# jolibrain/jolineedle

Hardware: AMD Instinct MI355X
Metric: glimpse-patches/sec (448px, seq-len 20) REINFORCE step (higher is better)
Workload: dtype f32; 1 GPU; configs[2]/[3]: REINFORCE rollout, gpt-nano + yolox-nano encoder, 448px, seq-len 20, --enable-stop, 64 agents/GPU x 1 GPU, 4480x4480 synthetic images, forced non-STOP actions (S=T); global_batch=64, seq_len=20

## Files before the change

include/jnroll.h:

```cpp
#ifndef JNROLL_H
#define JNROLL_H

#include <stddef.h>
#include <stdint.h>

#ifdef __cplusplus
extern "C" {
#endif

#define JN_ABI_VERSION 2

enum {
  JN_OK = 0,
  JN_EINVAL = -1,
  JN_ENOMEM = -2,
  JN_EHIP = -3,
  JN_ENOTFOUND = -4,
  JN_ESTATE = -5
};

enum { JN_MODE_GREEDY = 0, JN_MODE_SAMPLE = 1, JN_MODE_FORCED = 2 };

enum { JN_NET_GPT_BACKBONE = 0, JN_NET_DETECTOR = 1 };

typedef struct jn_ctx jn_ctx;

typedef struct jn_config {
  int32_t struct_size;
  int32_t device;
  int32_t n_layer, n_head, n_embd;
  int32_t block_size;
  int32_t n_actions;
  int32_t patch_size;
  int32_t use_pos_emb;
  int32_t no_patch_emb;
  int32_t concat_emb;
  int32_t decoder_pos_encoding;
  int32_t pos_emb_size;
  float gpt_bb_depth, gpt_bb_width;
  int32_t gpt_bb_depthwise;
  int32_t with_detector;
  float det_depth, det_width;
  int32_t det_depthwise;
  float det_conf_threshold;
  float det_nms_threshold;
  int32_t max_batch;
  int32_t max_det_per_patch;
  int32_t act_dtype;
  int32_t gpt_wide;
} jn_config;

typedef struct jn_tensor {
  const char* name;
  const void* data;
  int32_t dtype;
  int32_t ndim;
  int64_t shape[4];
} jn_tensor;

typedef struct jn_param_info {
  char name[160];
  int32_t dtype;
  int32_t ndim;
  int64_t shape[4];
  int32_t is_buffer;
  int32_t used;
} jn_param_info;

typedef struct jn_rollout_out {
  float* rewards_dev;
  float* returns_dev;
  float* logprobs_dev;
  float* entropies_dev;
  uint8_t* masks_dev;
  uint8_t* logit_masks_dev;
  int64_t* positions_dev;
  int64_t* actions_dev;
  float* logits_dev;
  float* final_emb_dev;
  float* patches_dev;
  float* det_boxes_dev;
  int32_t* det_counts_dev;
} jn_rollout_out;

int jn_abi_version(void);
const char* jn_last_error(void);
int jn_create(const jn_config* cfg, jn_ctx** out);
int jn_destroy(jn_ctx* ctx);

int jn_param_count(const jn_ctx* ctx);
int jn_param_info_at(const jn_ctx* ctx, int index, jn_param_info* out);
int jn_debug_forward_plan(const jn_ctx* ctx, int net, int N, int train, int with_head, int first_op, int32_t* out,
                          int cap);
int jn_debug_decision_route(const jn_ctx* ctx);
int jn_load_weights(jn_ctx* ctx, const jn_tensor* tensors, size_t n);

int jn_env_init(jn_ctx* ctx, const float* images_dev, const int64_t* bboxes_dev,
                int B, int H, int W, int nb, int max_ep_len, int stop_enabled, void* stream);
int jn_env_init_u8(jn_ctx* ctx, const uint8_t* images_dev, const int64_t* bboxes_dev,
                   int B, int H, int W, int nb, int max_ep_len, int stop_enabled, void* stream);
int jn_env_reset(jn_ctx* ctx, const int64_t* positions_dev, uint64_t seed, void* stream);
int jn_env_step(jn_ctx* ctx, const int64_t* actions_dev, float* rewards_dev,
                uint8_t* terminated_dev, uint8_t* truncated_dev, void* stream);
int jn_env_state(jn_ctx* ctx, int what, void** ptr_dev);
int jn_env_patches(jn_ctx* ctx, float* out_dev, void* stream);
int jn_gather_patches(const float* images_dev, const int64_t* positions_dev, float* out_dev,
                      int B, int C, int H, int W, int P, void* stream);
int jn_gather_patches_u8(const uint8_t* images_dev, const int64_t* positions_dev, float* out_dev,
                         int B, int C, int H, int W, int P, void* stream);
int jn_gather_patches_indexed(const float* images_dev, const int64_t* image_index_dev,
                              const int64_t* positions_dev, float* out_dev, int N, int n_images,
                              int C, int H, int W, int P, void* stream);
int jn_gather_patches_indexed_u8(const uint8_t* images_dev, const int64_t* image_index_dev,
                                 const int64_t* positions_dev, float* out_dev, int N, int n_images,
                                 int C, int H, int W, int P, void* stream);

typedef struct jn_image_view {
  const void* src;
  int32_t src_u8;
  int32_t Hs, Ws;
  int32_t rot;
  int32_t ty, tx;
} jn_image_view;
int jn_env_init_views(jn_ctx* ctx, const jn_image_view* views_host, const int64_t* bboxes_dev, int B, int Hc, int Wc,
                      int nb, int max_ep_len, int stop_enabled, void* stream);
int jn_env_init_ragged(jn_ctx* ctx, const jn_image_view* views_host, const int32_t* extents_host,
                       const int64_t* bboxes_dev, int B, int Hc, int Wc, int nb, int max_ep_len, int stop_enabled,
                       void* stream);
int jn_detection_cells(const int64_t* bboxes_dev, const int32_t* extents_dev, int B, int nb, int Gh, int Gw, int P,
                       int sample_neg, uint64_t seed, int capacity, int64_t* cells_dev, int64_t* targets_dev,
                       int32_t* offsets_dev, int32_t* n_pos_dev, void* stream);
int jn_rollout_boxes_to_image(const float* det_boxes_dev, const int32_t* det_counts_dev, const int64_t* positions_dev,
                              const uint8_t* masks_dev, int B, int T, int S, int K, int P, float* out_boxes_dev,
                              int32_t* out_totals_dev, void* stream);
int jn_merge_boxes(const float* boxes_dev, const int32_t* counts_dev, int B, int Nmax, int W, int target, float threshold,
                   float* out_boxes_dev, int32_t* out_counts_dev, int32_t* rounds_dev, void* stream);
int jn_yolox_loss(const float* raw_dev, const float* targets_dev, int N, int nb, int P, int stride0, int stride1,
                  int stride2, int use_l1, float loss_scale, float* d_raw_dev, float* metrics_dev, float* scale_dev,
                  void* stream);
int jn_yolox_loss_wide(const float* raw_dev, const float* targets_dev, int N, int nb, int P, int stride0, int stride1,
                       int stride2, int use_l1, float loss_scale, float* d_raw_dev, float* metrics_dev, float* scale_dev,
                       void* stream);
int jn_postprocess(const float* raw_dev, int N, int A, float conf_threshold, float nms_threshold, float clamp_max,
                   int max_out, float* boxes_dev, int32_t* counts_dev, int32_t* stats_dev, void* stream);
int jn_postprocess_all(const float* raw_dev, int N, int A, float conf_threshold, float nms_threshold, float clamp_max,
                       int max_out, float* boxes_dev, int32_t* counts_dev, int32_t* stats_dev, void* stream);
int jn_supervised_metrics(const float* logits_dev, const int64_t* current_actions_dev, const int64_t* next_actions_dev,
                          const uint8_t* masks_dev, int B, int T, int nA, float stop_weight, int on_self_trajectory,
                          float* token_loss_out_dev, uint8_t* predicted_out_dev, float* metrics_dev, void* stream);
int jn_match_detections(const float* preds_dev, const int32_t* pred_counts_dev, int B, int Nmax, int W,
                        const float* targets_dev, const int32_t* target_counts_dev, int Mmax, int max_det,
                        double* scores_dev, int32_t* hits_dev, int32_t* sel_dev, int32_t* n_pred_dev, int32_t* n_gt_dev,
                        void* stream);
int jn_average_precision(const double* scores_dev, const int32_t* hits_dev, const int32_t* n_pred_dev,
                         const int32_t* n_gt_dev, int B, int max_det, int pooled, const double* thresholds_dev,
                         int n_thresholds, double* out_dev, void* stream);
int jn_average_precision_segments(const double* scores_dev, const int32_t* hits_dev, const int32_t* n_pred_dev,
                                  const int32_t* n_gt_dev, int U, int max_det, const int32_t* seg_offsets_dev, int NS,
                                  int max_units, const double* thresholds_dev, int n_thresholds, double* out_dev, void* stream);
int jn_pool_walk_detections(const float* det_boxes_dev, const int32_t* det_counts_dev, const int64_t* positions_dev,
                            const int32_t* walk_tokens_dev, const int32_t* walk_first_dev, const int32_t* walk_count_dev, int A,
                            int T, int S, int K_det, int NI, int max_walks, int Gh, int Gw, int max_per_cell,
                            float* cell_boxes_dev, int32_t* cell_counts_dev, int32_t* cell_stats_dev, uint8_t* visited_dev,
                            void* stream);
int jn_gather_patches_views(const jn_image_view* views_dev, int n_views, const int64_t* image_index_dev,
                            const int64_t* positions_dev, void* out_dev, int out_u8, int N, int Hc, int Wc, int P,
                            void* stream);

#define JN_AUG_NPARAM 20
int jn_augment_patches(const float* in_dev, float* out_dev, const float* params_dev, const float* noise_dev,
                       uint64_t seed, int N, int P, void* stream);

int jn_backbone_forward(jn_ctx* ctx, int net, const float* patches_dev, int N, int train,
                        float* fpn0_dev, float* fpn1_dev, float* fpn2_dev, void* stream);
int jn_read_tensor(jn_ctx* ctx, const char* name, float* host_out, size_t numel);
int jn_embed_patches(jn_ctx* ctx, const float* patches_dev, int N, float* out_dev, void* stream);
int jn_zero_grad(jn_ctx* ctx, void* stream);
int jn_backbone_backward(jn_ctx* ctx, int net, const float* patches_dev, int N, const float* g0_dev,
                         const float* g1_dev, const float* g2_dev, void* stream);
typedef struct jn_train_opts {
  int32_t struct_size;
  int32_t reward_norm;
  float ret_mean, ret_std;
  float entropy_weight;
  float loss_scale;
} jn_train_opts;

int jn_reinforce_step(jn_ctx* ctx, int mode, const int64_t* forced_actions_dev,
                      const int64_t* start_positions_dev, uint64_t seed, int stop_early,
                      const jn_train_opts* opts, const jn_rollout_out* out, float* metrics_dev, void* stream);
int jn_reinforce_forward(jn_ctx* ctx, int mode, const int64_t* forced_actions_dev, const int64_t* start_positions_dev,
                         uint64_t seed, int stop_early, const jn_rollout_out* out, void* stream);
int jn_reinforce_backward(jn_ctx* ctx, const float* dlogprobs_dev, const float* dentropies_dev, void* stream);
int jn_set_activation_slots(jn_ctx* ctx, int n);
int jn_activation_slots_info(const jn_ctx* ctx, int net, int* act_slots, int* table_slots, size_t* slot_bytes, int* replayed_steps);
int jn_replay_chunks(int S, int act_slots, int g_slots, int* t0, int* n, int cap);
int jn_debug_replay_diff(jn_ctx* ctx, int step, long long* n_diff, void* stream);
int jn_arena_segment(jn_ctx* ctx, const char* name, size_t* off, size_t* numel);
int jn_export_arena(jn_ctx* ctx, int what, float* dst_dev, size_t numel, int accumulate, void* stream);
int jn_import_arena(jn_ctx* ctx, int what, const float* src_dev, size_t numel, void* stream);

int jn_set_dropout(jn_ctx* ctx, float p, uint64_t seed);
int jn_set_freeze(jn_ctx* ctx, int freeze_detector_backbone);
int jn_optimizer_steps(jn_ctx* ctx, int group, int* steps, int set);

int jn_supervised_step(jn_ctx* ctx, const float* patches_dev, const int64_t* current_actions_dev,
                       const int64_t* next_actions_dev, const int64_t* classes_dev, const int64_t* positions_dev,
                       const uint8_t* masks_dev, int B, int T, float stop_weight, float* logits_out_dev,
                       float* metrics_dev, void* stream);
int jn_supervised_forward(jn_ctx* ctx, const float* patches_dev, const int64_t* current_actions_dev,
                          const int64_t* classes_dev, const int64_t* positions_dev, int B, int T, float* logits_out_dev,
                          float* final_emb_out_dev, void* stream);
int jn_supervised_backward(jn_ctx* ctx, const float* dlogits_dev, void* stream);
int jn_gpt_backward_route(int C, int n_head, int T, int decision_route);
int jn_gpt_attention_backward(int form, const float* QKV_dev, const float* dY_dev, int B, int n_head, int C, int Lm, int L,
                              float pdrop, uint64_t seed, int layer, int Tmax, float* ATT_dev, float* Y_dev, float* dQKV_dev,
                              void* stream);
int jn_supervised_eval(jn_ctx* ctx, const float* patches_dev, const int64_t* current_actions_dev,
                       const int64_t* next_actions_dev, const int64_t* classes_dev, const int64_t* positions_dev,
                       const uint8_t* masks_dev, int B, int T, float stop_weight, int on_self_trajectory,
                       float* logits_out_dev, float* token_loss_out_dev, uint8_t* predicted_out_dev, float* metrics_dev,
                       void* stream);
int jn_optimizer_step(jn_ctx* ctx, float lr, float weight_decay, float clip_value, float grad_scale, void* stream);
int jn_arena_info(jn_ctx* ctx, size_t* total_numel, size_t* optim_gpt_numel);
int jn_set_grad_arena(jn_ctx* ctx, float* grads_dev, size_t numel);
int jn_read_param(jn_ctx* ctx, const char* name, float* host_out, size_t numel);
int jn_read_grad(jn_ctx* ctx, const char* name, float* host_out, size_t numel);

int jn_gpt_forward(jn_ctx* ctx, const float* patches_dev, const int64_t* actions_dev, const int64_t* classes_dev,
                   const int64_t* positions_dev, const float* prev_emb_dev, int B, int T, int Tp,
                   float* logits_dev, float* final_emb_dev, void* stream);
int jn_detect(jn_ctx* ctx, const float* patches_dev, int N, float* boxes_dev,
              int32_t* counts_dev, float* raw_dev, void* stream);
int jn_set_det_candidates(jn_ctx* ctx, int all);

int jn_detector_step(jn_ctx* ctx, const float* patches_dev, int N, const float* targets_dev, int nb,
                     float loss_scale, float* metrics_dev, void* stream);
#define JN_DETLOSS_MAX_BOXES 1024
int jn_set_det_loss_boxes(jn_ctx* ctx, int all);
int jn_detector_forward(jn_ctx* ctx, const float* patches_dev, int N, const float* targets_dev, int nb, int pass,
                        int n_pass, float* metrics_dev, float* boxes_dev, int32_t* counts_dev, float* fpn0_dev,
                        float* fpn1_dev, float* fpn2_dev, void* stream);
int jn_detector_backward(jn_ctx* ctx, int pass, const float* dloss_dev, float scale, void* stream);
int jn_detector_eval_loss(jn_ctx* ctx, const float* patches_dev, int N, const float* targets_dev, int nb,
                          float* metrics_dev, float* boxes_dev, int32_t* counts_dev, float* fpn0_dev, float* fpn1_dev,
                          float* fpn2_dev, void* stream);
int jn_optimizer_step_group(jn_ctx* ctx, int group, float lr, float weight_decay, float clip_value,
                            float grad_scale, void* stream);

int jn_rollout(jn_ctx* ctx, int mode, const int64_t* forced_actions_dev,
               const int64_t* start_positions_dev, uint64_t seed, int do_detection,
               int stop_early, const jn_rollout_out* out, void* stream);
int jn_set_rollout_positions(jn_ctx* ctx, int by_token);
int jn_teacher_actions(const int64_t* positions_dev, const uint8_t* visited_dev, const uint8_t* targets_dev, int B, int Gh,
                       int Gw, uint8_t* sets_dev, void* stream);
int jn_teacher_walks(const int64_t* bboxes_dev, const int64_t* start_positions_dev, int B, int nb, int Gh, int Gw, int P,
                     int T, int min_keypoints, int max_keypoints, int binomial_keypoints, uint64_t seed, int capacity,
                     int64_t* positions_dev, int64_t* current_actions_dev, int64_t* next_actions_dev, int64_t* labels_dev,
                     float* masks_dev, float* local_bboxes_dev, int32_t* n_steps_dev, uint8_t* targets_dev,
                     int64_t* cells_dev, float* bboxes_yolox_dev, int32_t* offsets_dev, void* stream);
int jn_pw_bwd_fused(const float* g_dev, const float* z_dev, const float* x_dev, const float* tab_dev, const float* save_dev,
                    const float* consts_dev, const float* w_dev, const float* gadd_dev, int accumulate, float* gx_dev,
                    float* gw_dev, int S, long long M, int cout, int cin, int route, int max_wg, void* stream);
int jn_conv3(const void* in_dev, int in_ld, const float* tab_dev, const float* w_dev, void* out_dev, int out_ld, int N, int H,
             int W, int cin, int cout, int stride, int transposed, int accumulate, double* stats_dev, const int* skip_flag_dev,
             int skip_when, int n_slots, long long in_slot_stride, long long out_slot_stride, int route, void* stream);
int jn_conv3_bwd_data_s2(const float* gz_dev, int g_ld, const float* w_dev, float* gin_dev, int gin_ld, int N, int H, int W, int cout,
                         int cin, int accumulate, int n_slots, int route, void* stream);
int jn_conv3_bwd_weight(const float* gz_dev, int g_ld, const float* x_dev, int x_ld, const float* tab_dev, float* gw_dev, int N, int H,
                        int W, int cout, int cin, int stride, int n_slots, int route, int max_wg, void* stream);
int jn_conv3_route(int kind, int N, int H, int W, int cin, int cout, int stride, int n_slots, int ld_a, int ld_b);
int jn_dw3x3(const void* in_dev, int in_ld, const float* tab_dev, const float* w_dev, void* out_dev, int out_ld, int N, int H, int W,
             int C, int stride, int dtype, double* stats_dev, const int* skip_flag_dev, int skip_when, int nrep, int route, void* stream);
int jn_dw3x3_route(int N, int C, int stride, int dtype);
int jn_dwpw(const void* in_dev, int in_ld, const float* itab_dev, const float* w_dw_dev, const float* mtab_dev, const float* w_pw_dev,
            void* out_dev, int out_ld, const void* res_dev, int res_ld, const float* rtab_dev, const float* ptab_dev, int N, int H, int W,
            int C, int cout, int stride, int dtype, const int* skip_flag_dev, int skip_when, void* stream);
int jn_dw_bwd(const float* g_dev, int g_ld, const float* z_dev, int z_ld, const float* x_dev, int x_ld, const float* otab_dev,
              const float* itab_dev, const float* save_dev, const float* consts_dev, const float* w_dev, float* gin_dev, int gin_ld,
              int accumulate, float* gw_dev, double* red_out_dev, int N, int H, int W, int C, int stride, int n_slots, int route,
              int use_wpart, float* wpart_back_dev, int max_wg, void* stream);
typedef struct jn_pw_run { int32_t c0, c1, stat0, g0, b0; float hw; } jn_pw_run;
typedef struct jn_pw_defer {
  const double* sums_dev; long long rep_stride; const float* params_dev;
  int32_t dN; long long dmax;
  int32_t n_runs, use_runs;
  jn_pw_run run[4];
} jn_pw_defer;
int jn_pw(const void* in_dev, int in_ld, int dtype_in, const float* tab_dev, const jn_pw_defer* defer, const float* w_dev,
          const float* bias_dev, void* out_dev, int out_ld, int dtype_out, int N, int H, int W, int cin, int cout, int bf16_mfma,
          int transposed, int in_identity, int accumulate, int act, double* stats_dev, int nrep, const int* skip_flag_dev, int skip_when,
          int n_slots, long long in_slot_stride, long long out_slot_stride, long long tab_slot_stride, float* up_out_dev, int up_ld,
          int route, int max_wg, void* stream);
int jn_pw_route(int N, int H, int W, int cin, int cout, int in_ld, int out_ld, int dtype_in, int dtype_out, int bf16_mfma, int transposed,
                int accumulate, int has_bias, int act, int n_slots, int has_up, int route, int32_t* variant_out);
int jn_pw_bwd_data_x3(const float* gz_dev, int g_ld, const float* w_dev, float* gx_dev, int gx_ld, long long M, int cout, int cin,
                      int n_slots, int max_wg, void* stream);
int jn_pw_bwd_weight(const float* gz_dev, int g_ld, const float* x_dev, int x_ld, const float* tab_dev, float* gw_dev, long long M, int cout,
                     int cin, int n_slots, long long gz_slot_stride, int use_wpart, float* wpart_back_dev, int exact, void* stream);
int jn_pw_bwd_weight_route(int cout, int cin);
int jn_stem(const void* src_dev, int src_u8, const int64_t* positions_dev, int pos_stride, long long sample_stride, long long chan_stride,
            int row_stride, int P, int N, int cout, const float* w_dev, void* out_dev, int out_ld, int out_dtype, double* stats_dev, int nrep,
            const int* skip_flag_dev, int skip_when, int max_wg, void* stream);
int jn_stem_bwd_weight(const void* src_dev, int src_u8, const int64_t* positions_dev, int pos_stride, long long pos_slot_stride,
                       long long sample_stride, long long chan_stride, int row_stride, int P, int N, int cout, const float* g_dev, int g_ld,
                       const float* z_dev, int z_ld, const float* otab_dev, const float* save_dev, const float* consts_dev, float* gw_dev,
                       float* wpart_dev, int n_slots, int max_wg, void* stream);
int jn_spp_route(int dtype, int ld, int h, int H, int W, int N, int bwd);
int jn_spp(void* cat_dev, int dtype, int ld, int h, int H, int W, int N, const float* tab_dev, const int* skip_flag_dev, int skip_when,
           int route, void* stream);
int jn_spp_bwd(const float* cat_dev, float* gcat_dev, int ld, int h, int H, int W, int N, const float* tab_dev, int n_slots, int route,
               void* stream);
int jn_upsample(const void* in_dev, int in_ld, void* out_dev, int out_ld, int dtype, int C, int H, int W, int N, const int* skip_flag_dev,
                int skip_when, void* stream);
int jn_upsample_bwd(const float* gdst_dev, int dst_ld, float* gsrc_dev, int src_ld, int C, int H, int W, int N, int accumulate, int n_slots,
                    void* stream);
int jn_addact(const void* z_dev, int z_ld, const float* ztab_dev, const void* res_dev, int res_ld, const float* rtab_dev, void* out_dev,
              int out_ld, int dtype, int C, long long M, const int* skip_flag_dev, int skip_when, void* stream);
int jn_bn_finalize(const double* stats_dev, long long rep_stride, double count, const float* gamma_dev, const float* beta_dev, float* run_mean_dev,
                   float* run_var_dev, float* save_dev, float* tab0_dev, float* tab1_dev, int C, float eps, float momentum,
                   const int* skip_flag_dev, int skip_when, void* stream);
int jn_bn_finalize_all(const double* stats_dev, long long rep_stride, int n_stat, int N, const float* hw_dev, const int* goff_dev,
                       const int* boff_dev, const float* params_dev, const int* t0_dev, const int* t1_dev, float* tab_dev, int tab_channels,
                       float* save_dev, float* run_mean_dev, float* run_var_dev, float eps, float momentum, const int* skip_flag_dev, int skip_when,
                       long long defer_max_m, void* stream);
int jn_bn_bwd_sums(const float* g_dev, int g_ld, const float* z_dev, int z_ld, const float* tab_dev, const float* save_dev, int C, long long M,
                   int n_slots, double* red_dev, const float* gamma_dev, const float* beta_dev, float* consts_dev, float* g_gamma_dev,
                   float* g_beta_dev, int reduce, int raw_moment, void* stream);
int jn_efpn_linear(const float* e_dev, const float* wt_dev, float* part_dev, int N, int K, int Co, int KS, const int* skip_flag_dev, int skip_when,
                   void* stream);
int jn_reinforce_loss(const float* logits_dev, const int64_t* actions_dev, const float* returns_dev, const float* rewards_dev,
                      const uint8_t* logit_masks_dev, const int32_t* n_done_dev, int B, int T, int nA, int reward_norm, float ret_mean,
                      float ret_std, float entropy_weight, float loss_scale, float* dlogits_dev, float* metrics_dev, void* stream);
int jn_logits_grad(const float* logits_dev, const int64_t* actions_dev, const float* dlogprobs_dev, const float* dentropies_dev,
                   const int32_t* n_done_dev, int B, int T, int nA, float* dlogits_dev, void* stream);
int jn_ce_loss(const float* logits_dev, const int64_t* target_dev, const uint8_t* masks_dev, int B, int T, int nA, float stop_weight,
               float* dlogits_dev, float* metrics_dev, void* stream);
int jn_adamw(float* p_dev, const float* g_dev, float* m_dev, float* v_dev, long long n, float lr, float weight_decay, int step, float clip_value,
             float grad_scale, void* stream);
int jn_set_rollout_teacher(jn_ctx* ctx, const uint8_t* targets_dev, uint8_t* sets_dev);
int jn_set_rollout_keys(jn_ctx* ctx, const uint64_t* keys_host, int n);
int jn_set_rollout_classes(jn_ctx* ctx, const int64_t* classes_host, int n);
int jn_rollout_steps(jn_ctx* ctx, int* n_steps, void* stream);

int jn_last_timing(jn_ctx* ctx, int what, float* ms);
int jn_set_profiling(jn_ctx* ctx, int enabled);

#ifdef __cplusplus
}
#endif
#endif
```

jolineedle_amd/_lib.py:

```python
import ctypes as C
import os
from pathlib import Path

_LIB = None
LIB_PATH = Path(__file__).resolve().parent / "lib" / "libjnroll.so"

JN_MODE_GREEDY, JN_MODE_SAMPLE, JN_MODE_FORCED = 0, 1, 2
JN_NET_GPT_BACKBONE, JN_NET_DETECTOR = 0, 1


class LibraryNotBuilt(RuntimeError):
    pass


class JnError(RuntimeError):
    pass


class JnConfig(C.Structure):
    _fields_ = [("struct_size", C.c_int32), ("device", C.c_int32),
                ("n_layer", C.c_int32), ("n_head", C.c_int32), ("n_embd", C.c_int32),
                ("block_size", C.c_int32), ("n_actions", C.c_int32), ("patch_size", C.c_int32),
                ("use_pos_emb", C.c_int32), ("no_patch_emb", C.c_int32), ("concat_emb", C.c_int32),
                ("decoder_pos_encoding", C.c_int32), ("pos_emb_size", C.c_int32),
                ("gpt_bb_depth", C.c_float), ("gpt_bb_width", C.c_float), ("gpt_bb_depthwise", C.c_int32),
                ("with_detector", C.c_int32), ("det_depth", C.c_float), ("det_width", C.c_float),
                ("det_depthwise", C.c_int32), ("det_conf_threshold", C.c_float),
                ("det_nms_threshold", C.c_float), ("max_batch", C.c_int32), ("max_det_per_patch", C.c_int32),
                ("act_dtype", C.c_int32), ("gpt_wide", C.c_int32)]


class JnTensor(C.Structure):
    _fields_ = [("name", C.c_char_p), ("data", C.c_void_p), ("dtype", C.c_int32), ("ndim", C.c_int32),
                ("shape", C.c_int64 * 4)]


class JnParamInfo(C.Structure):
    _fields_ = [("name", C.c_char * 160), ("dtype", C.c_int32), ("ndim", C.c_int32),
                ("shape", C.c_int64 * 4), ("is_buffer", C.c_int32), ("used", C.c_int32)]


class JnTrainOpts(C.Structure):
    _fields_ = [("struct_size", C.c_int32), ("reward_norm", C.c_int32), ("ret_mean", C.c_float),
                ("ret_std", C.c_float), ("entropy_weight", C.c_float), ("loss_scale", C.c_float)]


class JnRolloutOut(C.Structure):
    _fields_ = [(n, C.c_void_p) for n in (
        "rewards_dev", "returns_dev", "logprobs_dev", "entropies_dev", "masks_dev", "logit_masks_dev",
        "positions_dev", "actions_dev", "logits_dev", "final_emb_dev", "patches_dev", "det_boxes_dev",
        "det_counts_dev")]


class JnImageView(C.Structure):
    _fields_ = [("src", C.c_void_p), ("src_u8", C.c_int32), ("Hs", C.c_int32), ("Ws", C.c_int32), ("rot", C.c_int32),
                ("ty", C.c_int32), ("tx", C.c_int32)]


class JnPwRun(C.Structure):
    _fields_ = [("c0", C.c_int32), ("c1", C.c_int32), ("stat0", C.c_int32), ("g0", C.c_int32), ("b0", C.c_int32), ("hw", C.c_float)]


class JnPwDefer(C.Structure):
    _fields_ = [("sums_dev", C.c_void_p), ("rep_stride", C.c_longlong), ("params_dev", C.c_void_p), ("dN", C.c_int32),
                ("dmax", C.c_longlong), ("n_runs", C.c_int32), ("use_runs", C.c_int32), ("run", JnPwRun * 4)]


ABI_VERSION = 2

SIGNATURES = {
    "jn_abi_version": (C.c_int, []),
    "jn_last_error": (C.c_char_p, []),
    "jn_create": (C.c_int, [C.POINTER(JnConfig), C.POINTER(C.c_void_p)]),
    "jn_destroy": (C.c_int, [C.c_void_p]),
    "jn_param_count": (C.c_int, [C.c_void_p]),
    "jn_param_info_at": (C.c_int, [C.c_void_p, C.c_int, C.POINTER(JnParamInfo)]),
    "jn_debug_forward_plan": (C.c_int, [C.c_void_p, C.c_int, C.c_int, C.c_int, C.c_int, C.c_int, C.POINTER(C.c_int32), C.c_int]),
    "jn_debug_decision_route": (C.c_int, [C.c_void_p]),
    "jn_load_weights": (C.c_int, [C.c_void_p, C.POINTER(JnTensor), C.c_size_t]),
    "jn_env_init": (C.c_int, [C.c_void_p, C.c_void_p, C.c_void_p, C.c_int, C.c_int, C.c_int, C.c_int, C.c_int,
                              C.c_int, C.c_void_p]),
    "jn_env_init_u8": (C.c_int, [C.c_void_p, C.c_void_p, C.c_void_p, C.c_int, C.c_int, C.c_int, C.c_int, C.c_int,
                                 C.c_int, C.c_void_p]),
    "jn_env_reset": (C.c_int, [C.c_void_p, C.c_void_p, C.c_uint64, C.c_void_p]),
    "jn_env_step": (C.c_int, [C.c_void_p, C.c_void_p, C.c_void_p, C.c_void_p, C.c_void_p, C.c_void_p]),
    "jn_env_state": (C.c_int, [C.c_void_p, C.c_int, C.POINTER(C.c_void_p)]),
    "jn_env_patches": (C.c_int, [C.c_void_p, C.c_void_p, C.c_void_p]),
    "jn_gather_patches": (C.c_int, [C.c_void_p, C.c_void_p, C.c_void_p, C.c_int, C.c_int, C.c_int, C.c_int,
                                    C.c_int, C.c_void_p]),
    "jn_gather_patches_u8": (C.c_int, [C.c_void_p, C.c_void_p, C.c_void_p, C.c_int, C.c_int, C.c_int, C.c_int,
                                       C.c_int, C.c_void_p]),
    "jn_augment_patches": (C.c_int, [C.c_void_p, C.c_void_p, C.c_void_p, C.c_void_p, C.c_uint64, C.c_int, C.c_int, C.c_void_p]),
    "jn_gather_patches_indexed": (C.c_int, [C.c_void_p, C.c_void_p, C.c_void_p, C.c_void_p, C.c_int, C.c_int, C.c_int,
                                            C.c_int, C.c_int, C.c_int, C.c_void_p]),
    "jn_gather_patches_indexed_u8": (C.c_int, [C.c_void_p, C.c_void_p, C.c_void_p, C.c_void_p, C.c_int, C.c_int,
                                               C.c_int, C.c_int, C.c_int, C.c_int, C.c_void_p]),
    "jn_env_init_views": (C.c_int, [C.c_void_p, C.POINTER(JnImageView), C.c_void_p, C.c_int, C.c_int, C.c_int, C.c_int, C.c_int,
                                    C.c_int, C.c_void_p]),
    "jn_env_init_ragged": (C.c_int, [C.c_void_p, C.POINTER(JnImageView), C.POINTER(C.c_int32), C.c_void_p, C.c_int, C.c_int, C.c_int,
                                     C.c_int, C.c_int, C.c_int, C.c_void_p]),
    "jn_rollout_boxes_to_image": (C.c_int, [C.c_void_p, C.c_void_p, C.c_void_p, C.c_void_p, C.c_int, C.c_int, C.c_int, C.c_int,
                                            C.c_int, C.c_void_p, C.c_void_p, C.c_void_p]),
    "jn_merge_boxes": (C.c_int, [C.c_void_p, C.c_void_p, C.c_int, C.c_int, C.c_int, C.c_int, C.c_float, C.c_void_p, C.c_void_p,
                                 C.c_void_p, C.c_void_p]),
    "jn_yolox_loss": (C.c_int, [C.c_void_p, C.c_void_p, C.c_int, C.c_int, C.c_int, C.c_int, C.c_int, C.c_int, C.c_int, C.c_float,
                                C.c_void_p, C.c_void_p, C.c_void_p, C.c_void_p]),
    "jn_yolox_loss_wide": (C.c_int, [C.c_void_p, C.c_void_p, C.c_int, C.c_int, C.c_int, C.c_int, C.c_int, C.c_int, C.c_int, C.c_float,
                                     C.c_void_p, C.c_void_p, C.c_void_p, C.c_void_p]),
    "jn_postprocess": (C.c_int, [C.c_void_p, C.c_int, C.c_int, C.c_float, C.c_float, C.c_float, C.c_int, C.c_void_p, C.c_void_p,
                                 C.c_void_p, C.c_void_p]),
    "jn_postprocess_all": (C.c_int, [C.c_void_p, C.c_int, C.c_int, C.c_float, C.c_float, C.c_float, C.c_int, C.c_void_p, C.c_void_p,
                                     C.c_void_p, C.c_void_p]),
    "jn_match_detections": (C.c_int, [C.c_void_p, C.c_void_p, C.c_int, C.c_int, C.c_int, C.c_void_p, C.c_void_p, C.c_int, C.c_int,
                                      C.c_void_p, C.c_void_p, C.c_void_p, C.c_void_p, C.c_void_p, C.c_void_p]),
    "jn_average_precision": (C.c_int, [C.c_void_p, C.c_void_p, C.c_void_p, C.c_void_p, C.c_int, C.c_int, C.c_int, C.c_void_p,
                                       C.c_int, C.c_void_p, C.c_void_p]),
    "jn_average_precision_segments": (C.c_int, [C.c_void_p, C.c_void_p, C.c_void_p, C.c_void_p, C.c_int, C.c_int, C.c_void_p,
                                                C.c_int, C.c_int, C.c_void_p, C.c_int, C.c_void_p, C.c_void_p]),
    "jn_pool_walk_detections": (C.c_int, [C.c_void_p] * 6 + [C.c_int] * 9 + [C.c_void_p] * 5),
    "jn_detection_cells": (C.c_int, [C.c_void_p, C.c_void_p] + [C.c_int] * 6 + [C.c_uint64, C.c_int] + [C.c_void_p] * 5),
    "jn_gather_patches_views": (C.c_int, [C.c_void_p, C.c_int, C.c_void_p, C.c_void_p, C.c_void_p, C.c_int, C.c_int, C.c_int,
                                          C.c_int, C.c_int, C.c_void_p]),
    "jn_backbone_forward": (C.c_int, [C.c_void_p, C.c_int, C.c_void_p, C.c_int, C.c_int, C.c_void_p, C.c_void_p,
                                      C.c_void_p, C.c_void_p]),
    "jn_read_tensor": (C.c_int, [C.c_void_p, C.c_char_p, C.c_void_p, C.c_size_t]),
    "jn_embed_patches": (C.c_int, [C.c_void_p, C.c_void_p, C.c_int, C.c_void_p, C.c_void_p]),
    "jn_reinforce_step": (C.c_int, [C.c_void_p, C.c_int, C.c_void_p, C.c_void_p, C.c_uint64, C.c_int,
                                    C.POINTER(JnTrainOpts), C.POINTER(JnRolloutOut), C.c_void_p, C.c_void_p]),
    "jn_supervised_step": (C.c_int, [C.c_void_p, C.c_void_p, C.c_void_p, C.c_void_p, C.c_void_p, C.c_void_p, C.c_void_p,
                                     C.c_int, C.c_int, C.c_float, C.c_void_p, C.c_void_p, C.c_void_p]),
    "jn_supervised_forward": (C.c_int, [C.c_void_p, C.c_void_p, C.c_void_p, C.c_void_p, C.c_void_p, C.c_int, C.c_int,
                                        C.c_void_p, C.c_void_p, C.c_void_p]),
    "jn_supervised_backward": (C.c_int, [C.c_void_p, C.c_void_p, C.c_void_p]),
    "jn_gpt_backward_route": (C.c_int, [C.c_int] * 4),
    "jn_gpt_attention_backward": (C.c_int, [C.c_int, C.c_void_p, C.c_void_p] + [C.c_int] * 5 + [C.c_float, C.c_uint64, C.c_int, C.c_int] +
                                           [C.c_void_p] * 4),
    "jn_optimizer_step": (C.c_int, [C.c_void_p, C.c_float, C.c_float, C.c_float, C.c_float, C.c_void_p]),
    "jn_arena_info": (C.c_int, [C.c_void_p, C.POINTER(C.c_size_t), C.POINTER(C.c_size_t)]),
    "jn_set_grad_arena": (C.c_int, [C.c_void_p, C.c_void_p, C.c_size_t]),
    "jn_read_param": (C.c_int, [C.c_void_p, C.c_char_p, C.c_void_p, C.c_size_t]),
    "jn_zero_grad": (C.c_int, [C.c_void_p, C.c_void_p]),
    "jn_backbone_backward": (C.c_int, [C.c_void_p, C.c_int, C.c_void_p, C.c_int, C.c_void_p, C.c_void_p, C.c_void_p,
                                       C.c_void_p]),
    "jn_read_grad": (C.c_int, [C.c_void_p, C.c_char_p, C.c_void_p, C.c_size_t]),
    "jn_gpt_forward": (C.c_int, [C.c_void_p, C.c_void_p, C.c_void_p, C.c_void_p, C.c_void_p, C.c_void_p, C.c_int, C.c_int,
                                 C.c_int, C.c_void_p, C.c_void_p, C.c_void_p]),
    "jn_detect": (C.c_int, [C.c_void_p, C.c_void_p, C.c_int, C.c_void_p, C.c_void_p, C.c_void_p, C.c_void_p]),
    "jn_set_det_candidates": (C.c_int, [C.c_void_p, C.c_int]),
    "jn_set_det_loss_boxes": (C.c_int, [C.c_void_p, C.c_int]),
    "jn_rollout": (C.c_int, [C.c_void_p, C.c_int, C.c_void_p, C.c_void_p, C.c_uint64, C.c_int, C.c_int,
                             C.POINTER(JnRolloutOut), C.c_void_p]),
    "jn_set_rollout_positions": (C.c_int, [C.c_void_p, C.c_int]),
    "jn_teacher_actions": (C.c_int, [C.c_void_p, C.c_void_p, C.c_void_p, C.c_int, C.c_int, C.c_int, C.c_void_p, C.c_void_p]),
    "jn_teacher_walks": (C.c_int, [C.c_void_p, C.c_void_p] + [C.c_int] * 9 + [C.c_uint64, C.c_int] + [C.c_void_p] * 12),
    "jn_pw_bwd_fused": (C.c_int, [C.c_void_p] * 8 + [C.c_int] + [C.c_void_p] * 2 + [C.c_int, C.c_longlong] + [C.c_int] * 4 + [C.c_void_p]),
    "jn_conv3": (C.c_int, [C.c_void_p, C.c_int, C.c_void_p, C.c_void_p, C.c_void_p] + [C.c_int] * 9 + [C.c_void_p, C.c_void_p, C.c_int, C.c_int,
                           C.c_longlong, C.c_longlong, C.c_int, C.c_void_p]),
    "jn_conv3_bwd_data_s2": (C.c_int, [C.c_void_p, C.c_int, C.c_void_p, C.c_void_p] + [C.c_int] * 9 + [C.c_void_p]),
    "jn_conv3_bwd_weight": (C.c_int, [C.c_void_p, C.c_int, C.c_void_p, C.c_int, C.c_void_p, C.c_void_p] + [C.c_int] * 9 + [C.c_void_p]),
    "jn_conv3_route": (C.c_int, [C.c_int] * 10),
    "jn_dw3x3": (C.c_int, [C.c_void_p, C.c_int, C.c_void_p, C.c_void_p, C.c_void_p] + [C.c_int] * 7 + [C.c_void_p, C.c_void_p] + [C.c_int] * 3 +
                          [C.c_void_p]),
    "jn_dw3x3_route": (C.c_int, [C.c_int] * 4),
    "jn_dwpw": (C.c_int, [C.c_void_p, C.c_int] + [C.c_void_p] * 5 + [C.c_int, C.c_void_p, C.c_int, C.c_void_p, C.c_void_p] + [C.c_int] * 7 +
                         [C.c_void_p, C.c_int, C.c_void_p]),
    "jn_dw_bwd": (C.c_int, [C.c_void_p, C.c_int] * 3 + [C.c_void_p] * 6 + [C.c_int, C.c_int, C.c_void_p, C.c_void_p] + [C.c_int] * 8 +
                           [C.c_void_p, C.c_int, C.c_void_p]),
    "jn_pw": (C.c_int, [C.c_void_p, C.c_int, C.c_int, C.c_void_p, C.c_void_p, C.c_void_p, C.c_void_p, C.c_void_p, C.c_int, C.c_int] + [C.c_int] * 10 +
                       [C.c_void_p, C.c_int, C.c_void_p, C.c_int, C.c_int, C.c_longlong, C.c_longlong, C.c_longlong, C.c_void_p, C.c_int, C.c_int,
                        C.c_int, C.c_void_p]),
    "jn_pw_route": (C.c_int, [C.c_int] * 17 + [C.c_void_p]),
    "jn_pw_bwd_weight_route": (C.c_int, [C.c_int] * 2),
    "jn_pw_bwd_data_x3": (C.c_int, [C.c_void_p, C.c_int, C.c_void_p, C.c_void_p, C.c_int, C.c_longlong, C.c_int, C.c_int, C.c_int, C.c_int,
                                    C.c_void_p]),
    "jn_pw_bwd_weight": (C.c_int, [C.c_void_p, C.c_int, C.c_void_p, C.c_int, C.c_void_p, C.c_void_p, C.c_longlong, C.c_int, C.c_int, C.c_int,
                                   C.c_longlong, C.c_int, C.c_void_p, C.c_int, C.c_void_p]),
    "jn_stem": (C.c_int, [C.c_void_p, C.c_int, C.c_void_p, C.c_int, C.c_longlong, C.c_longlong] + [C.c_int] * 4 + [C.c_void_p, C.c_void_p, C.c_int,
                          C.c_int, C.c_void_p, C.c_int, C.c_void_p, C.c_int, C.c_int, C.c_void_p]),
    "jn_stem_bwd_weight": (C.c_int, [C.c_void_p, C.c_int, C.c_void_p, C.c_int, C.c_longlong, C.c_longlong, C.c_longlong] + [C.c_int] * 4 +
                                     [C.c_void_p, C.c_int, C.c_void_p, C.c_int] + [C.c_void_p] * 5 + [C.c_int, C.c_int, C.c_void_p]),
    "jn_spp_route": (C.c_int, [C.c_int] * 7),
    "jn_spp": (C.c_int, [C.c_void_p] + [C.c_int] * 6 + [C.c_void_p, C.c_void_p, C.c_int, C.c_int, C.c_void_p]),
    "jn_spp_bwd": (C.c_int, [C.c_void_p, C.c_void_p] + [C.c_int] * 5 + [C.c_void_p, C.c_int, C.c_int, C.c_void_p]),
    "jn_upsample": (C.c_int, [C.c_void_p, C.c_int, C.c_void_p, C.c_int] + [C.c_int] * 5 + [C.c_void_p, C.c_int, C.c_void_p]),
    "jn_upsample_bwd": (C.c_int, [C.c_void_p, C.c_int, C.c_void_p, C.c_int] + [C.c_int] * 6 + [C.c_void_p]),
    "jn_addact": (C.c_int, [C.c_void_p, C.c_int, C.c_void_p] * 2 + [C.c_void_p, C.c_int, C.c_int, C.c_int, C.c_longlong, C.c_void_p, C.c_int,
                            C.c_void_p]),
    "jn_bn_finalize": (C.c_int, [C.c_void_p, C.c_longlong, C.c_double] + [C.c_void_p] * 7 + [C.c_int, C.c_float, C.c_float, C.c_void_p, C.c_int,
                                 C.c_void_p]),
    "jn_bn_finalize_all": (C.c_int, [C.c_void_p, C.c_longlong, C.c_int, C.c_int] + [C.c_void_p] * 7 + [C.c_int] + [C.c_void_p] * 3 +
                                     [C.c_float, C.c_float, C.c_void_p, C.c_int, C.c_longlong, C.c_void_p]),
    "jn_bn_bwd_sums": (C.c_int, [C.c_void_p, C.c_int, C.c_void_p, C.c_int, C.c_void_p, C.c_void_p, C.c_int, C.c_longlong, C.c_int] +
                                 [C.c_void_p] * 6 + [C.c_int, C.c_int, C.c_void_p]),
    "jn_efpn_linear": (C.c_int, [C.c_void_p] * 3 + [C.c_int] * 4 + [C.c_void_p, C.c_int, C.c_void_p]),
    "jn_reinforce_loss": (C.c_int, [C.c_void_p] * 6 + [C.c_int] * 4 + [C.c_float] * 4 + [C.c_void_p] * 3),
    "jn_logits_grad": (C.c_int, [C.c_void_p] * 5 + [C.c_int] * 3 + [C.c_void_p] * 2),
    "jn_ce_loss": (C.c_int, [C.c_void_p] * 3 + [C.c_int] * 3 + [C.c_float] + [C.c_void_p] * 3),
    "jn_adamw": (C.c_int, [C.c_void_p] * 4 + [C.c_longlong, C.c_float, C.c_float, C.c_int, C.c_float, C.c_float, C.c_void_p]),
    "jn_set_rollout_teacher":(C.c_int, [C.c_void_p, C.c_void_p, C.c_void_p]),
    "jn_set_rollout_keys": (C.c_int, [C.c_void_p, C.c_void_p, C.c_int]),
    "jn_set_rollout_classes": (C.c_int, [C.c_void_p, C.c_void_p, C.c_int]),
    "jn_rollout_steps": (C.c_int, [C.c_void_p, C.POINTER(C.c_int), C.c_void_p]),
    "jn_last_timing": (C.c_int, [C.c_void_p, C.c_int, C.POINTER(C.c_float)]),
    "jn_set_profiling": (C.c_int, [C.c_void_p, C.c_int]),
    "jn_detector_step": (C.c_int, [C.c_void_p, C.c_void_p, C.c_int, C.c_void_p, C.c_int, C.c_float, C.c_void_p, C.c_void_p]),
    "jn_detector_forward": (C.c_int, [C.c_void_p, C.c_void_p, C.c_int, C.c_void_p, C.c_int, C.c_int, C.c_int, C.c_void_p,
                                      C.c_void_p, C.c_void_p, C.c_void_p, C.c_void_p, C.c_void_p, C.c_void_p]),
    "jn_detector_backward": (C.c_int, [C.c_void_p, C.c_int, C.c_void_p, C.c_float, C.c_void_p]),
    "jn_optimizer_step_group": (C.c_int, [C.c_void_p, C.c_int, C.c_float, C.c_float, C.c_float, C.c_float, C.c_void_p]),
    "jn_reinforce_forward": (C.c_int, [C.c_void_p, C.c_int, C.c_void_p, C.c_void_p, C.c_uint64, C.c_int,
                                       C.POINTER(JnRolloutOut), C.c_void_p]),
    "jn_reinforce_backward": (C.c_int, [C.c_void_p, C.c_void_p, C.c_void_p, C.c_void_p]),
    "jn_set_activation_slots": (C.c_int, [C.c_void_p, C.c_int]),
    "jn_activation_slots_info": (C.c_int, [C.c_void_p, C.c_int, C.POINTER(C.c_int), C.POINTER(C.c_int), C.POINTER(C.c_size_t),
                                           C.POINTER(C.c_int)]),
    "jn_replay_chunks": (C.c_int, [C.c_int, C.c_int, C.c_int, C.POINTER(C.c_int), C.POINTER(C.c_int), C.c_int]),
    "jn_debug_replay_diff": (C.c_int, [C.c_void_p, C.c_int, C.POINTER(C.c_longlong), C.c_void_p]),
    "jn_arena_segment": (C.c_int, [C.c_void_p, C.c_char_p, C.POINTER(C.c_size_t), C.POINTER(C.c_size_t)]),
    "jn_export_arena": (C.c_int, [C.c_void_p, C.c_int, C.c_void_p, C.c_size_t, C.c_int, C.c_void_p]),
    "jn_import_arena": (C.c_int, [C.c_void_p, C.c_int, C.c_void_p, C.c_size_t, C.c_void_p]),
    "jn_set_dropout": (C.c_int, [C.c_void_p, C.c_float, C.c_uint64]),
    "jn_set_freeze": (C.c_int, [C.c_void_p, C.c_int]),
    "jn_optimizer_steps": (C.c_int, [C.c_void_p, C.c_int, C.POINTER(C.c_int), C.c_int]),
    "jn_supervised_metrics": (C.c_int, [C.c_void_p, C.c_void_p, C.c_void_p, C.c_void_p, C.c_int, C.c_int, C.c_int, C.c_float, C.c_int,
                                        C.c_void_p, C.c_void_p, C.c_void_p, C.c_void_p]),
    "jn_supervised_eval": (C.c_int, [C.c_void_p] * 7 + [C.c_int, C.c_int, C.c_float, C.c_int] + [C.c_void_p] * 5),
    "jn_detector_eval_loss": (C.c_int, [C.c_void_p, C.c_void_p, C.c_int, C.c_void_p, C.c_int] + [C.c_void_p] * 7),
}


def load_library(path=None):
    global _LIB
    if _LIB is not None and path is None:
        return _LIB
    p = Path(path or os.environ.get("JNROLL_LIB", LIB_PATH))
    if not p.exists():
        raise LibraryNotBuilt(
            f"{p} not found: the HIP extension is not built. Run `bash jolineedle_amd/csrc/build.sh` "
            "(or __graft_entry__.build()). There is no CPU fallback for this path.")
    lib = C.CDLL(str(p))
    for name, (res, args) in SIGNATURES.items():
        fn = getattr(lib, name)
        fn.restype, fn.argtypes = res, args
    if lib.jn_abi_version() != ABI_VERSION:
        raise JnError(f"libjnroll ABI {lib.jn_abi_version()} != {ABI_VERSION}")
    if path is None:
        _LIB = lib
    return lib


def check(rc, what=""):
    if rc != 0:
        msg = load_library().jn_last_error().decode(errors="replace")
        raise JnError(f"{what} failed with code {rc}: {msg}")


def ptr(t):
    return None if t is None else C.c_void_p(t.data_ptr())


def current_stream(device):
    import torch
    return C.c_void_p(torch.cuda.current_stream(device).cuda_stream)
```

jolineedle_amd/csrc/api_kernels.hip:

```cpp
#include <cstring>

#include "jn_internal.h"

using namespace jnr;

static ChanTab chan_tab(const float* tab, long long C, int c0 = 0) {
  float* p = const_cast<float*>(tab) + c0;
  ChanTab t{};
  t.sc = p; t.sh = p + C; t.fl = p + 2 * C;
  return t;
}

static bool map_ok(int N, int H, int W) { return N >= 1 && H >= 1 && W >= 1 && (long long)N * H * W <= (1 << 24); }
static bool pixels_ok(long long M) { return M >= 1 && M <= (1 << 24); }
static bool quad_chan_ok(int C) { return C >= 4 && C % 4 == 0 && C <= 4096; }
static bool ld_ok(int ld, int C) { return ld >= C && ld <= 8192; }
static bool quad_ld_ok(int ld, int C) { return ld_ok(ld, C) && ld % 4 == 0; }
static bool slots_ok(int n_slots) { return n_slots >= 1 && n_slots <= 64; }
static bool dtype_ok(int dtype) { return dtype == JN_F32 || dtype == JN_BF16; }

class Scratch {
 public:
  explicit Scratch(hipStream_t s) : s_(s) {}
  Scratch(const Scratch&) = delete;
  ~Scratch() {
    if (p_) { (void)hipStreamSynchronize(s_); (void)hipFree(p_); }
  }
  hipError_t take(size_t bytes) { return hipMalloc(&p_, bytes); }
  template <typename T>
  T* as() const { return static_cast<T*>(p_); }
 private:
  hipStream_t s_;
  void* p_ = nullptr;
};

struct SlotLayout {
  int S;
  hipStream_t s;
  hipError_t in(float* field, size_t slot, const float* dense, size_t n) const {
    return hipMemcpy2DAsync(field, slot * sizeof(float), dense, n * sizeof(float), n * sizeof(float), S, hipMemcpyDeviceToDevice, s);
  }
  hipError_t back(float* dense, size_t n, const float* field, size_t slot) const {
    return hipMemcpy2DAsync(dense, n * sizeof(float), field, slot * sizeof(float), n * sizeof(float), S, hipMemcpyDeviceToDevice, s);
  }
};

static const auto nothing_back = [] { return hipSuccess; };
template <bool HostRefusal = false, typename L, typename B = decltype(nothing_back)>
static int run_entry(const char* who, hipStream_t s, L launch, const char* refusal = "the launcher refused the arguments", B back = nothing_back) {
  const int rc = launch();
  if (HostRefusal) JN_CHECK(rc == 0, JN_EINVAL, "%s: %s", who, refusal);
  hipError_t e = hipGetLastError();
  if (e == hipSuccess) e = back();
  if (e == hipSuccess) e = hipStreamSynchronize(s);
  JN_CHECK(e == hipSuccess, JN_EHIP, "%s: the launch, the copy back or the wait for the stream failed: %s", who, hipGetErrorString(e));
  JN_CHECK(rc == 0, JN_EINVAL, "%s: %s", who, refusal);
  return JN_OK;
}

extern "C" {

int jn_pw_bwd_fused(const float* g_dev, const float* z_dev, const float* x_dev, const float* tab_dev, const float* save_dev,
                    const float* consts_dev, const float* w_dev, const float* gadd_dev, int accumulate, float* gx_dev,
                    float* gw_dev, int S, long long M, int cout, int cin, int route, int max_wg, void* stream) {
  JN_CHECK(g_dev && z_dev && x_dev && tab_dev && save_dev && consts_dev && w_dev && gx_dev && gw_dev, JN_EINVAL,
           "jn_pw_bwd_fused: null argument");
  JN_CHECK(S >= 1 && M >= 1 && M <= (1LL << 40), JN_EINVAL, "jn_pw_bwd_fused: S=%d M=%lld", S, M);
  JN_CHECK(cout >= 16 && cin >= 16 && pw_bwd_fused_supported(cout, cin), JN_EINVAL, "jn_pw_bwd_fused: %d -> %d channels: no fused kernel",
           cin, cout);
  JN_CHECK((route == 0 || route == 1) && max_wg >= 0, JN_EINVAL, "jn_pw_bwd_fused: route=%d max_wg=%d", route, max_wg);
  hipStream_t s = (hipStream_t)stream;
  const long long C = cout + cin;
  const size_t zn = (size_t)M * cout, xn = (size_t)M * cin, act = zn + xn, grad = zn + 2 * xn;
  Scratch scratch(s);
  JN_HIP(scratch.take(((size_t)S * (act + grad) + (size_t)2 * cout * cin) * sizeof(float)));
  float* ws = scratch.as<float>();
  float *za = ws, *xa = za + zn, *ga = ws + (size_t)S * act, *gxa = ga + zn, *gadda = gxa + xn, *w_frag = ws + (size_t)S * (act + grad);
  const SlotLayout lay{S, s};
  JN_HIP(lay.in(za, act, z_dev, zn));
  JN_HIP(lay.in(xa, act, x_dev, xn));
  JN_HIP(lay.in(ga, grad, g_dev, zn));
  if (accumulate) JN_HIP(lay.in(gxa, grad, gx_dev, xn));
  if (gadd_dev) JN_HIP(lay.in(gadda, grad, gadd_dev, xn));
  PwBwdFusedArgs a{};
  a.g = ga; a.g_ld = cout; a.z = za; a.z_ld = cout;
  a.ot = chan_tab(tab_dev, C);
  a.save = save_dev; a.consts = consts_dev;
  a.x = xa; a.x_ld = cin;
  a.it = chan_tab(tab_dev, C, cout);
  a.w = w_dev; a.gx = gxa; a.gx_ld = cin; a.accumulate = accumulate ? 1 : 0; a.gw = gw_dev;
  a.M = M; a.cout = cout; a.cin = cin;
  a.sb.n = S; a.sb.act = (long long)act; a.sb.grad = (long long)grad; a.sb.tab = 3 * C; a.sb.save = 2LL * cout; a.sb.consts = 3LL * cout;
  if (gadd_dev) { a.gadd = gadda; a.gadd_ld = cin; }
  a.w_frag = w_frag; a.route = route; a.max_wg = max_wg;
  return run_entry("jn_pw_bwd_fused", s, [&] { return launch_pw_bwd_fused(a, s); }, "no fused kernel took the launch",
                   [&] { return lay.back(gx_dev, xn, gxa, grad); });
}

}

static bool conv3_shape_ok(int N, int H, int W, int cin, int cout, int stride, int n_slots, int ld_a, int c_a, int ld_b, int c_b) {
  return map_ok(N, H, W) && quad_chan_ok(cin) && quad_chan_ok(cout) && (stride == 1 || (stride == 2 && H % 2 == 0 && W % 2 == 0)) &&
         slots_ok(n_slots) && quad_ld_ok(ld_a, c_a) && quad_ld_ok(ld_b, c_b);
}

static ConvArgs conv3_entry_args(int N, int H, int W, int cin, int cout, int stride, int transposed, int in_ld, int out_ld,
                                 int n_slots, int dtype) {
  ConvArgs a{};
  a.in_ld = in_ld; a.in_dtype = dtype; a.out_ld = out_ld; a.out_dtype = dtype; a.bf16_mfma = dtype == JN_BF16;
  a.N = N; a.H = H; a.W = W; a.OH = H / stride; a.OW = W / stride; a.cin = cin; a.cout = cout; a.stride = stride; a.act = ACT_NONE;
  a.w_transposed = transposed ? 1 : 0; a.n_slots = n_slots;
  return a;
}

extern "C" {

int jn_conv3_route(int kind, int N, int H, int W, int cin, int cout, int stride, int n_slots, int ld_a, int ld_b) {
  JN_CHECK(kind >= 0 && kind <= 3, JN_EINVAL, "jn_conv3_route: kind=%d", kind);
  const bool fwd_like = kind <= 1;
  JN_CHECK(conv3_shape_ok(N, H, W, cin, cout, stride, n_slots, ld_a, fwd_like ? cin : cout, ld_b, fwd_like ? cout : cin) &&
               (kind != 1 || stride == 1) && (kind != 2 || stride == 2),
           JN_EINVAL, "jn_conv3_route: kind %d, %d x %d x %d, %d -> %d channels, stride %d, %d slots, leading dimensions %d and %d", kind, N,
           H, W, cin, cout, stride, n_slots, ld_a, ld_b);
  int r;
  if (fwd_like) {
    ConvArgs a = conv3_entry_args(N, H, W, cin, cout, stride, kind == 1, ld_a, ld_b, n_slots, JN_F32);
    r = conv3_route(a, 0);
  } else if (kind == 2) {
    r = conv3_bwd_data_s2_route(ld_a, ld_b, H / 2, W / 2, cout, cin, N, n_slots, 0);
  } else {
    r = conv3_bwd_weight_route(ld_a, ld_b, cout, cin, 0);
  }
  JN_CHECK(r > 0, JN_EINVAL, "jn_conv3_route: no dense 3x3 kernel takes this launch");
  return r;
}

int jn_conv3(const void* in_dev, int in_ld, const float* tab_dev, const float* w_dev, void* out_dev, int out_ld, int N, int H,
             int W, int cin, int cout, int stride, int transposed, int accumulate, double* stats_dev, const int* skip_flag_dev,
             int skip_when, int n_slots, long long in_slot_stride, long long out_slot_stride, int route, void* stream) {
  JN_CHECK(in_dev && tab_dev && w_dev && out_dev, JN_EINVAL, "jn_conv3: null argument");
  JN_CHECK(conv3_shape_ok(N, H, W, cin, cout, stride, n_slots, in_ld, cin, out_ld, cout) && (!transposed || stride == 1), JN_EINVAL,
           "jn_conv3: %d x %d x %d, %d -> %d channels, stride %d, transposed %d, %d slots, leading dimensions %d and %d", N, H, W, cin, cout,
           stride, transposed, n_slots, in_ld, out_ld);
  const int OH = H / stride, OW = W / stride;
  JN_CHECK(route >= 0 && route <= C3_ROUTE_BF16 && in_slot_stride >= 0 && out_slot_stride >= 0 &&
               (n_slots == 1 || (in_slot_stride >= (long long)N * H * W * in_ld && out_slot_stride >= (long long)N * OH * OW * out_ld &&
                                 in_slot_stride % 4 == 0 && out_slot_stride % 4 == 0)),
           JN_EINVAL, "jn_conv3: route=%d, slot strides %lld and %lld", route, in_slot_stride, out_slot_stride);
  const bool bf16 = route == C3_ROUTE_BF16;
  JN_CHECK(!bf16 || n_slots == 1, JN_EINVAL, "jn_conv3: the bf16 kernel takes one slot");
  ConvArgs a = conv3_entry_args(N, H, W, cin, cout, stride, transposed, in_ld, out_ld, n_slots, bf16 ? JN_BF16 : JN_F32);
  a.in = in_dev; a.itab = chan_tab(tab_dev, cin); a.w = w_dev; a.out = out_dev;
  a.accumulate = accumulate ? 1 : 0; a.stats = stats_dev; a.stats_rep_stride = 2LL * cout; a.skip_flag = skip_flag_dev; a.skip_when = skip_when;
  a.in_slot_stride = in_slot_stride; a.out_slot_stride = out_slot_stride;
  if (bf16) a.w_bf16 = w_dev;
  JN_CHECK(conv3_route(a, route) > 0, JN_EINVAL, "jn_conv3: route %d does not take this launch", route);
  hipStream_t s = (hipStream_t)stream;
  Scratch wb(s);
  if (bf16) {
    const size_t n = (size_t)9 * cout * cin;
    std::vector<float> hw(n);
    std::vector<uint16_t> hb(n);
    JN_HIP(hipMemcpy(hw.data(), w_dev, n * sizeof(float), hipMemcpyDeviceToHost));
    for (size_t i = 0; i < n; ++i) {
      uint32_t u;
      std::memcpy(&u, &hw[i], 4);
      u += 0x7FFFu + ((u >> 16) & 1u);
      hb[i] = (uint16_t)(u >> 16);
    }
    JN_HIP(wb.take(n * sizeof(uint16_t)));
    JN_HIP(hipMemcpy(wb.as<uint16_t>(), hb.data(), n * sizeof(uint16_t), hipMemcpyHostToDevice));
    a.w_bf16 = wb.as<uint16_t>();
  }
  return run_entry("jn_conv3", s, [&] { return launch_conv3(a, s, route); }, "the kernel's LDS was refused");
}

int jn_conv3_bwd_data_s2(const float* gz_dev, int g_ld, const float* w_dev, float* gin_dev, int gin_ld, int N, int H, int W, int cout,
                         int cin, int accumulate, int n_slots, int route, void* stream) {
  JN_CHECK(gz_dev && w_dev && gin_dev, JN_EINVAL, "jn_conv3_bwd_data_s2: null argument");
  JN_CHECK(conv3_shape_ok(N, H, W, cin, cout, 2, n_slots, g_ld, cout, gin_ld, cin), JN_EINVAL,
           "jn_conv3_bwd_data_s2: %d x %d x %d, %d -> %d channels, %d slots, leading dimensions %d and %d", N, H, W, cin, cout, n_slots, g_ld,
           gin_ld);
  const int OH = H / 2, OW = W / 2;
  JN_CHECK(route >= 0 && route <= C3_ROUTE_X3 && conv3_bwd_data_s2_route(g_ld, gin_ld, OH, OW, cout, cin, N, n_slots, route) > 0, JN_EINVAL,
           "jn_conv3_bwd_data_s2: route %d does not take this launch", route);
  hipStream_t s = (hipStream_t)stream;
  const size_t gn = (size_t)N * OH * OW * g_ld, xn = (size_t)N * H * W * gin_ld, slot = gn + xn;
  Scratch scratch(s);
  JN_HIP(scratch.take((size_t)n_slots * slot * sizeof(float)));
  float *ga = scratch.as<float>(), *gina = ga + gn;
  const SlotLayout lay{n_slots, s};
  JN_HIP(lay.in(ga, slot, gz_dev, gn));
  JN_HIP(lay.in(gina, slot, gin_dev, xn));
  SlotBatch sb;
  sb.n = n_slots; sb.grad = (long long)slot;
  auto launch = [&] { return launch_conv3_bwd_data_s2(ga, g_ld, w_dev, gina, gin_ld, H, W, OH, OW, cout, cin, N, accumulate ? 1 : 0, s, sb, route); };
  return run_entry("jn_conv3_bwd_data_s2", s, launch, "the kernel's LDS was refused", [&] { return lay.back(gin_dev, xn, gina, slot); });
}

int jn_conv3_bwd_weight(const float* gz_dev, int g_ld, const float* x_dev, int x_ld, const float* tab_dev, float* gw_dev, int N, int H,
                        int W, int cout, int cin, int stride, int n_slots, int route, int max_wg, void* stream) {
  JN_CHECK(gz_dev && x_dev && tab_dev && gw_dev, JN_EINVAL, "jn_conv3_bwd_weight: null argument");
  JN_CHECK(conv3_shape_ok(N, H, W, cin, cout, stride, n_slots, g_ld, cout, x_ld, cin), JN_EINVAL,
           "jn_conv3_bwd_weight: %d x %d x %d, %d -> %d channels, stride %d, %d slots, leading dimensions %d and %d", N, H, W, cin, cout,
           stride, n_slots, g_ld, x_ld);
  JN_CHECK(route >= 0 && route <= CW_ROUTE_EXACT && max_wg >= 0 && conv3_bwd_weight_route(g_ld, x_ld, cout, cin, route) > 0, JN_EINVAL,
           "jn_conv3_bwd_weight: route=%d max_wg=%d does not take this launch", route, max_wg);
  const int OH = H / stride, OW = W / stride;
  hipStream_t s = (hipStream_t)stream;
  const ChanTab it = chan_tab(tab_dev, cin);
  SlotBatch sb;
  sb.n = n_slots; sb.grad = (long long)N * OH * OW * g_ld; sb.act = (long long)N * H * W * x_ld; sb.tab = 3LL * cin;
  auto launch = [&] { return launch_conv3_bwd_weight(gz_dev, g_ld, x_dev, x_ld, it, gw_dev, H, W, OH, OW, cout, cin, N, stride, s, sb, route, max_wg); };
  return run_entry("jn_conv3_bwd_weight", s, launch, "the kernel's LDS was refused");
}

}

static bool dw_shape_ok(int N, int H, int W, int C, int stride) { return map_ok(N, H, W) && quad_chan_ok(C) && (stride == 1 || stride == 2); }

extern "C" {

int jn_dw3x3_route(int N, int C, int stride, int dtype) {
  JN_CHECK(dw_shape_ok(N, 1, 1, C, stride) && dtype_ok(dtype), JN_EINVAL, "jn_dw3x3_route: N=%d C=%d stride=%d dtype=%d", N, C, stride, dtype);
  ConvArgs a{};
  a.N = N; a.cin = a.cout = C; a.stride = stride; a.in_dtype = a.out_dtype = dtype;
  return dw_route(a, 0);
}

int jn_dw3x3(const void* in_dev, int in_ld, const float* tab_dev, const float* w_dev, void* out_dev, int out_ld, int N, int H, int W,
             int C, int stride, int dtype, double* stats_dev, const int* skip_flag_dev, int skip_when, int nrep, int route, void* stream) {
  JN_CHECK(in_dev && tab_dev && w_dev && out_dev, JN_EINVAL, "jn_dw3x3: null argument");
  JN_CHECK(dw_shape_ok(N, H, W, C, stride) && quad_ld_ok(in_ld, C) && quad_ld_ok(out_ld, C) && dtype_ok(dtype), JN_EINVAL,
           "jn_dw3x3: %d x %d x %d, %d channels, stride %d, dtype %d, leading dimensions %d and %d", N, H, W, C, stride, dtype, in_ld, out_ld);
  JN_CHECK(nrep >= 1 && nrep <= JN_NREP && route >= 0 && route <= DW_ROUTE_STRIP, JN_EINVAL, "jn_dw3x3: nrep=%d route=%d", nrep, route);
  ConvArgs a{};
  a.in = in_dev; a.in_ld = in_ld; a.in_dtype = dtype; a.itab = chan_tab(tab_dev, C); a.w = w_dev;
  a.out = out_dev; a.out_ld = out_ld; a.out_dtype = dtype;
  a.N = N; a.H = H; a.W = W; a.OH = (H + stride - 1) / stride; a.OW = (W + stride - 1) / stride; a.cin = a.cout = C; a.stride = stride;
  a.act = ACT_NONE; a.stats = stats_dev; a.stats_rep_stride = 2LL * C; a.stats_nrep = nrep;
  a.skip_flag = skip_flag_dev; a.skip_when = skip_when;
  JN_CHECK(dw_route(a, route) > 0, JN_EINVAL, "jn_dw3x3: route %d does not take this launch", route);
  hipStream_t s = (hipStream_t)stream;
  return run_entry("jn_dw3x3", s, [&] { return launch_dw(a, s, route); }, "no kernel took the launch");
}

int jn_dwpw(const void* in_dev, int in_ld, const float* itab_dev, const float* w_dw_dev, const float* mtab_dev, const float* w_pw_dev,
            void* out_dev, int out_ld, const void* res_dev, int res_ld, const float* rtab_dev, const float* ptab_dev, int N, int H, int W,
            int C, int cout, int stride, int dtype, const int* skip_flag_dev, int skip_when, void* stream) {
  JN_CHECK(in_dev && itab_dev && w_dw_dev && mtab_dev && w_pw_dev && out_dev, JN_EINVAL, "jn_dwpw: null argument");
  JN_CHECK(dw_shape_ok(N, H, W, C, stride) && quad_ld_ok(in_ld, C) && cout >= 4 && cout % 4 == 0 && quad_ld_ok(out_ld, cout) && dtype_ok(dtype),
           JN_EINVAL, "jn_dwpw: %d x %d x %d, %d -> %d channels, stride %d, dtype %d, leading dimensions %d and %d", N, H, W, C, cout, stride,
           dtype, in_ld, out_ld);
  JN_CHECK(dwpw_supported(C, cout, stride), JN_EINVAL, "jn_dwpw: %d -> %d channels at stride %d: no fused kernel", C, cout, stride);
  JN_CHECK(!res_dev || (rtab_dev && ptab_dev && quad_ld_ok(res_ld, cout)), JN_EINVAL, "jn_dwpw: a shortcut needs both tables and res_ld=%d >= %d",
           res_ld, cout);
  DwPwArgs f{};
  f.in = in_dev; f.in_ld = in_ld; f.itab = chan_tab(itab_dev, C); f.w_dw = w_dw_dev; f.mtab = chan_tab(mtab_dev, C); f.w_pw = w_pw_dev;
  f.out = out_dev; f.out_ld = out_ld; f.dtype = dtype; f.C = C; f.cout = cout; f.N = N; f.H = H; f.W = W;
  f.OH = (H + stride - 1) / stride; f.OW = (W + stride - 1) / stride; f.stride = stride; f.skip_flag = skip_flag_dev; f.skip_when = skip_when;
  if (res_dev) { f.res = res_dev; f.res_ld = res_ld; f.rtab = chan_tab(rtab_dev, cout); f.ptab = chan_tab(ptab_dev, cout); }
  hipStream_t s = (hipStream_t)stream;
  return run_entry("jn_dwpw", s, [&] { return launch_dwpw(f, s); }, "no kernel took the launch");
}

int jn_dw_bwd(const float* g_dev, int g_ld, const float* z_dev, int z_ld, const float* x_dev, int x_ld, const float* otab_dev,
              const float* itab_dev, const float* save_dev, const float* consts_dev, const float* w_dev, float* gin_dev, int gin_ld,
              int accumulate, float* gw_dev, double* red_out_dev, int N, int H, int W, int C, int stride, int n_slots, int route,
              int use_wpart, float* wpart_back_dev, int max_wg, void* stream) {
  JN_CHECK(g_dev && z_dev && x_dev && otab_dev && itab_dev && save_dev && consts_dev && w_dev && gin_dev && gw_dev, JN_EINVAL,
           "jn_dw_bwd: null argument");
  JN_CHECK(dw_shape_ok(N, H, W, C, stride) && slots_ok(n_slots) && quad_ld_ok(g_ld, C) && quad_ld_ok(z_ld, C) && quad_ld_ok(x_ld, C) &&
               quad_ld_ok(gin_ld, C),
           JN_EINVAL, "jn_dw_bwd: %d x %d x %d, %d channels, stride %d, %d slots, leading dimensions %d, %d, %d and %d", N, H, W, C, stride,
           n_slots, g_ld, z_ld, x_ld, gin_ld);
  JN_CHECK(route >= 0 && route <= 2 && max_wg >= 0 && (!use_wpart || wpart_back_dev), JN_EINVAL, "jn_dw_bwd: route=%d max_wg=%d use_wpart=%d",
           route, max_wg, use_wpart);
  const int OH = (H + stride - 1) / stride, OW = (W + stride - 1) / stride;
  const bool fused_ok = dw_bwd_fused_supported(C, H, W, OH, OW, stride);
  if (route == 0) route = fused_ok ? 1 : 2;
  JN_CHECK(route == 2 || fused_ok, JN_EINVAL, "jn_dw_bwd: the fused kernel takes whole blocks of 16 channels, not %d", C);
  JN_CHECK(!red_out_dev || (route == 1 && !accumulate), JN_EINVAL,
           "jn_dw_bwd: the input layer's sums are formed by the fused kernel only, from a gradient it writes (route %d, accumulate %d)", route,
           accumulate);
  hipStream_t s = (hipStream_t)stream;
  const size_t zn = (size_t)N * OH * OW * z_ld, xn = (size_t)N * H * W * x_ld, gn = (size_t)N * OH * OW * g_ld, gin_n = (size_t)N * H * W * gin_ld;
  const size_t act = zn + xn, grad = gn + gin_n, wp = use_wpart ? (size_t)JN_NREP * JN_WPART_MAX : 0;
  Scratch scratch(s);
  JN_HIP(scratch.take(((size_t)n_slots * (act + grad) + wp) * sizeof(float)));
  float* ws = scratch.as<float>();
  float *za = ws, *xa = za + zn, *ga = ws + (size_t)n_slots * act, *gina = ga + gn, *wpart = use_wpart ? ws + (size_t)n_slots * (act + grad) : nullptr;
  const SlotLayout lay{n_slots, s};
  JN_HIP(lay.in(za, act, z_dev, zn));
  JN_HIP(lay.in(xa, act, x_dev, xn));
  JN_HIP(lay.in(ga, grad, g_dev, gn));
  JN_HIP(lay.in(gina, grad, gin_dev, gin_n));
  if (wpart) JN_HIP(hipMemsetAsync(wpart, 0, wp * sizeof(float), s));
  SlotBatch sb;
  sb.n = n_slots; sb.act = (long long)act; sb.grad = (long long)grad; sb.tab = 3LL * C; sb.save = 2LL * C; sb.consts = 3LL * C;
  sb.red = (long long)JN_NREP * 2 * C;
  const ChanTab ot = chan_tab(otab_dev, C), it = chan_tab(itab_dev, C);
  auto launch = [&] {
    if (route == 1) {
      DwBwdFusedArgs fa{};
      fa.g = ga; fa.g_ld = g_ld; fa.z = za; fa.z_ld = z_ld; fa.ot = ot; fa.save = save_dev; fa.consts = consts_dev;
      fa.x = xa; fa.x_ld = x_ld; fa.it = it; fa.w = w_dev;
      fa.gin = gina; fa.gin_ld = gin_ld; fa.accumulate = accumulate ? 1 : 0; fa.gw = gw_dev; fa.wpart = wpart;
      fa.C = C; fa.H = H; fa.W = W; fa.OH = OH; fa.OW = OW; fa.N = N; fa.stride = stride; fa.sb = sb;
      fa.red_in = red_out_dev; fa.red_rep_stride = 2LL * C; fa.max_wg = max_wg;
      return launch_dw_bwd_fused(fa, s);
    }
    const long long M = (long long)N * OH * OW;
    int rc = launch_bn_bwd_gz(ga, g_ld, za, z_ld, ot, save_dev, consts_dev, C, M, s, sb);
    if (rc == 0) rc = launch_dw_bwd_data(ga, g_ld, w_dev, gina, gin_ld, C, H, W, OH, OW, N, stride, accumulate ? 1 : 0, s, sb);
    if (rc == 0) rc = launch_dw_bwd_weight(ga, g_ld, xa, x_ld, it, gw_dev, wpart, C, H, W, OH, OW, N, stride, s, sb, max_wg);
    return rc;
  };
  auto back = [&] {
    hipError_t e = lay.back(gin_dev, gin_n, gina, grad);
    if (e == hipSuccess && wpart) e = hipMemcpyAsync(wpart_back_dev, wpart, wp * sizeof(float), hipMemcpyDeviceToDevice, s);
    return e;
  };
  return run_entry("jn_dw_bwd", s, launch, "no kernel took the launch", back);
}

}

static bool pw_shape_ok(int N, int H, int W, int cin, int cout, int in_ld, int out_ld, int n_slots) {
  return map_ok(N, H, W) && quad_chan_ok(cin) && quad_chan_ok(cout) && quad_ld_ok(in_ld, cin) && quad_ld_ok(out_ld, cout) && slots_ok(n_slots);
}
static bool pw_flags_ok(int dtype_in, int dtype_out, int act) { return dtype_ok(dtype_in) && dtype_ok(dtype_out) && act >= ACT_NONE && act <= ACT_SIGMOID; }

static ConvArgs pw_entry_args(int N, int H, int W, int cin, int cout, int in_ld, int out_ld, int dtype_in, int dtype_out, int bf16_mfma,
                              int transposed, int in_identity, int accumulate, bool has_bias, int act, int n_slots, bool has_up, const void* some) {
  ConvArgs a{};
  a.in_ld = in_ld; a.in_dtype = dtype_in; a.out_ld = out_ld; a.out_dtype = dtype_out; a.bf16_mfma = bf16_mfma ? 1 : 0;
  a.N = N; a.H = a.OH = H; a.W = a.OW = W; a.cin = cin; a.cout = cout; a.stride = 1; a.act = act;
  a.accumulate = accumulate ? 1 : 0; a.w_transposed = transposed ? 1 : 0; a.in_identity = in_identity ? 1 : 0; a.n_slots = n_slots;
  a.bias = has_bias ? (const float*)some : nullptr; a.w_x3 = some; a.up_out = has_up ? const_cast<void*>(some) : nullptr;
  return a;
}

static bool pw_defer_ok(const jn_pw_defer* d, int cin) {
  if (!d->sums_dev || !d->params_dev || d->dN < 1 || d->dmax < 0 || d->n_runs < 1 || d->n_runs > 4 || d->rep_stride < 2) return false;
  int prev = 0;
  for (int i = 0; i < d->n_runs; ++i) {
    const jn_pw_run& r = d->run[i];
    if (r.c0 < prev || r.c1 <= r.c0 || r.c1 > cin || !(r.hw >= 1.0f)) return false;
    if (r.stat0 >= 0 && (r.g0 < 0 || r.b0 < 0 || 2LL * (r.stat0 + (r.c1 - r.c0)) > d->rep_stride)) return false;
    prev = r.c1;
  }
  return true;
}

static int pw_split_planes(const float* w_dev, char* ws, size_t plane_bytes, int cin, int cout, hipStream_t s) {
  const size_t nw = (size_t)cout * cin;
  launch_w_split3(w_dev, ws, (long long)nw, s);
  if (!pw_x3_fragment_order(cin, cout)) return JN_OK;
  const X3FragConv row{0, cout, cin};
  JN_HIP(hipMemcpyAsync(ws + plane_bytes, &row, sizeof(row), hipMemcpyHostToDevice, s));
  JN_HIP(hipStreamSynchronize(s));
  launch_w_split3_frag(w_dev, ws, (const X3FragConv*)(ws + plane_bytes), 1, (int)nw, s);
  return JN_OK;
}

static int pw_defer_table(ChanTab& t, const jn_pw_defer* defer, int cin, char* arr, hipStream_t s) {
  t.dparams = defer->params_dev; t.dstats = defer->sums_dev; t.drep_stride = defer->rep_stride; t.dN = defer->dN; t.dmax = defer->dmax;
  if (arr) {
    std::vector<int32_t> h(4 * (size_t)cin, -1);
    float* hw = reinterpret_cast<float*>(h.data() + cin);
    for (int c = 0; c < cin; ++c) { hw[c] = 0.0f; h[2 * cin + c] = h[3 * cin + c] = 0; }
    for (int i = 0; i < defer->n_runs; ++i) {
      const jn_pw_run& q = defer->run[i];
      for (int c = q.c0; c < q.c1; ++c) {
        h[c] = q.stat0 >= 0 ? q.stat0 + (c - q.c0) : -1; hw[c] = q.hw;
        h[2 * cin + c] = q.stat0 >= 0 ? q.g0 + (c - q.c0) : 0; h[3 * cin + c] = q.stat0 >= 0 ? q.b0 + (c - q.c0) : 0;
      }
    }
    JN_HIP(hipMemcpyAsync(arr, h.data(), h.size() * 4, hipMemcpyHostToDevice, s));
    JN_HIP(hipStreamSynchronize(s));
    t.dsrc = (const int*)arr; t.dhw = (const float*)(arr + 4 * (size_t)cin); t.dgoff = (const int*)(arr + 8 * (size_t)cin);
    t.dboff = (const int*)(arr + 12 * (size_t)cin);
    t.nseg = 0;
    return JN_OK;
  }
  t.dsrc = reinterpret_cast<const int*>(defer->sums_dev);
  t.nseg = defer->n_runs;
  ChanTab::Run* dst[4] = {&t.r0, &t.r1, &t.r2, &t.r3};
  for (int i = 0; i < defer->n_runs; ++i) {
    const jn_pw_run& q = defer->run[i];
    const bool deferred = q.stat0 >= 0 && (double)defer->dN * q.hw <= (double)defer->dmax;
    *dst[i] = ChanTab::Run{q.c0, q.c1, deferred ? q.stat0 : -1, q.g0, q.b0, q.hw};
  }
  return JN_OK;
}

extern "C" {

int jn_pw_route(int N, int H, int W, int cin, int cout, int in_ld, int out_ld, int dtype_in, int dtype_out, int bf16_mfma, int transposed,
// ... 363 lines not shown
```

jolineedle_amd/csrc/api_net.hip:

```cpp
#include <algorithm>
#include <cstring>

#include "jn_internal.h"

using namespace jnr;

extern "C"
__global__ void bn_eval_table_kernel(const float* __restrict__ gamma, const float* __restrict__ beta,
                                     const float* __restrict__ rmean, const float* __restrict__ rvar, ChanTab t0,
                                     ChanTab t1, int C, float eps) {
  const int c = blockIdx.x * blockDim.x + threadIdx.x;
  if (c >= C) return;
  const float sc = gamma[c] / sqrtf(rvar[c] + eps);
  const float sh = beta[c] - rmean[c] * sc;
  t0.sc[c] = sc; t0.sh[c] = sh; t0.fl[c] = 1.0f;
  if (t1.sc) { t1.sc[c] = sc; t1.sh[c] = sh; t1.fl[c] = 1.0f; }
}

extern "C"
__global__ void fill_kernel(float* p, float v, long long n) {
  const long long i = (long long)blockIdx.x * blockDim.x + threadIdx.x;
  if (i < n) p[i] = v;
}

// ... 446 lines not shown
  const int MB = ctx->cfg.max_batch;
  JN_CHECK(net.act_dtype == JN_F32, JN_ESTATE, "training needs act_dtype = fp32 (bf16 is the inference mode)");
  JN_CHECK(nsl >= 1 && nsl <= net.g_slots && slot >= 0 && slot + nsl <= net.a_slots && ts >= 0 && ts + nsl <= net.n_slots, JN_ESTATE,
           "backward over %d slots from %d (tables from %d): not allocated", nsl, slot, ts);
  std::vector<BwdStep> plan;
  int rc = plan_backward(net, with_head, fpn_zero, plan);
  if (rc) return rc;
  JN_HIP(hipMemsetAsync(net.bred, 0, (size_t)nsl * JN_NREP * 2 * net.stat_channels * sizeof(double), s));
  const long long rep_stride = 2LL * net.stat_channels;
  SlotBatch sb;
  sb.n = nsl;
  sb.act = (long long)net.per_image_floats * MB;
  sb.grad = (long long)net.per_image_floats * MB;
  sb.tab = 3LL * net.tab_channels;
  sb.save = 2LL * net.stat_channels;
  sb.red = (long long)JN_NREP * 2 * net.stat_channels;
  sb.consts = 3LL * net.stat_channels;
  sb.pos = pos_slot_stride;
  float* save = slot_save(net, ts);
  auto ptr = [&](const View& v) { return (const float*)view_ptr(net, slot, MB, v); };
  auto gptr = [&](const View& v) { return net.gact + net.buf_off[v.buf] * (size_t)MB + v.coff; };
  auto tab = [&](const View& v) { return view_tab(net, ts, v); };
  auto ld = [&](const View& v) { return net.bufs[v.buf].C; };
  auto sums = [&](int p, int half) {
    const ConvW& pcw = net.convs[net.ops[p].wslot];
    return net.bred + 2 * (pcw.stat_off + (half > 0 ? pcw.cout / 2 : 0));
  };
  const ChanTab ident{ctx->ident, ctx->ident + 2048, ctx->ident + 4096};
  static const bool no_aux = std::getenv("JN_NO_AUX_STREAM") != nullptr;
  static const bool dbg_plan = std::getenv("JN_DBG_BWD_PLAN") != nullptr;
  bool aux_used = false;
  if (!no_aux) { int ra = ensure_aux_stream(ctx); if (ra) return ra; }
  auto fork_aux = [&](hipStream_t& ws) -> int {
    ws = s;
    if (no_aux) return JN_OK;
    JN_HIP(hipEventRecord(ctx->aux_fork, s));
    JN_HIP(hipStreamWaitEvent(ctx->aux_stream, ctx->aux_fork, 0));
    ws = ctx->aux_stream;
    aux_used = true;
    return JN_OK;
  };
  struct ConvB { const Op& op; const BwdStep& st; const ConvW& cw; float* g; int g_ld; long long M; float* consts; float* gw; };
  auto bn_sums_consts = [&](const ConvB& c) -> int {
    const ConvW& cw = c.cw;
    const int parts = c.st.red_by && !cw.prefix2.empty() ? 2 : 1, h = cw.cout / parts;
    double* red = net.bred + 2 * cw.stat_off;
    if (dbg_plan) {
      const int hm = c.st.red_by;
      const long long sep = parts == 2 ? (c.M / N) * h * (2 - ((hm & 1) + ((hm >> 1) & 1))) : hm ? 0 : (c.M / N) * cw.cout;
      std::fprintf(stderr, "[bwd-plan] %-34s kind %d cout %4d cin %4d M/patch %6lld stride %d acc_in %d separate-reduce elements/patch %8lld%s\n",
                   c.op.name.c_str(), (int)c.op.kind, cw.cout, cw.cin, c.M / N, c.op.stride, (int)c.op.acc_in, sep,
                   parts == 2 ? (hm == 3 ? " (both halves by their consumers)" : " (one half by its consumer)") : "");
    }
    for (int part = 0; part < parts; ++part) {
      const int c0 = part * h, by_consumer = (c.st.red_by >> part) & 1;
      float* sv = save + 2 * (cw.stat_off + c0);
      JN_CHECK(by_consumer || launch_bn_bwd_reduce(c.g + c0, c.g_ld, ptr(c.op.out) + c0, ld(c.op.out), tab_at(tab(c.op.out), c0), sv, h, c.M,
                                                   red + 2 * c0, rep_stride, s, sb) == 0,
               JN_ESTATE, "launch_bn_bwd_reduce: %s has %d channels (whole quads, at most %d)", c.op.name.c_str(), h, JN_BN_BWD_MAX_C);
      JN_CHECK(launch_bn_bwd_consts(red + 2 * c0, rep_stride, (double)c.M, cw.gamma_dev + c0, cw.beta_dev + c0, sv, c.consts + 3 * c0,
                                    grad_of(ctx, cw.gamma_dev) + c0, grad_of(ctx, cw.beta_dev) + c0, h, s, sb, by_consumer) == 0,
               JN_ESTATE, "launch_bn_bwd_consts: %s was refused", c.op.name.c_str());
    }
    return JN_OK;
  };
  auto gz_conv_args = [&](const ConvB& c) {
    ConvArgs a{};
    a.in = c.g; a.in_ld = c.g_ld; a.in_dtype = JN_F32; a.itab = ident; a.w = c.cw.w_dev;
    a.out = gptr(c.op.in); a.out_ld = ld(c.op.in); a.out_dtype = JN_F32;
    a.N = N; a.H = c.op.out.H; a.W = c.op.out.W; a.OH = c.op.in.H; a.OW = c.op.in.W;
    a.cin = c.cw.cout; a.cout = c.cw.cin; a.stride = 1; a.act = ACT_NONE;
    a.accumulate = c.op.acc_in ? 1 : 0; a.w_transposed = 1; a.in_identity = 1;
    a.n_slots = nsl; a.in_slot_stride = sb.grad; a.out_slot_stride = sb.grad;
    return a;
  };
  auto bn_gz = [&](const ConvB& c) {
    launch_bn_bwd_gz(c.g, c.g_ld, ptr(c.op.out), ld(c.op.out), tab(c.op.out), save + 2 * c.cw.stat_off, c.consts, c.cw.cout, c.M,
                     s, sb);
  };
  const int n_ops_b = (int)plan.size();
  static const bool bwd_profile = std::getenv("JN_BWD_PROFILE") != nullptr;
  OpProfile prof(bwd_profile, n_ops_b + 1, s);
  prof.mark(n_ops_b);
  for (int obi = n_ops_b - 1; obi >= 0; --obi) {
    const Op& op = net.ops[obi];
    const BwdStep& st = plan[obi];
    const long long M = (long long)N * op.out.H * op.out.W;
    if (op.wslot < 0) {
      switch (st.route) {
        case BR_ADDACT_COPY: case BR_ADDACT_FOLD:
          JN_CHECK(!op.acc_in || launch_grad_copy(gptr(op.out), ld(op.out), gptr(op.in), ld(op.in), op.out.C, M, 1, s, sb) == 0, JN_ESTATE,
                   "launch_grad_copy: %s was refused", op.name.c_str());
          JN_CHECK(st.route != BR_ADDACT_COPY ||
                       launch_grad_copy(gptr(op.out), ld(op.out), gptr(op.res), ld(op.res), op.out.C, M, op.acc_res ? 1 : 0, s, sb) == 0,
                   JN_ESTATE, "launch_grad_copy: %s was refused", op.name.c_str());
          break;
        case BR_SPP: {
          const View full = net_full_view(net, op.out.buf);
          JN_CHECK(launch_spp_bwd(ptr(full), gptr(full), ld(op.out), op.in.C, op.in.H, op.in.W, N, tab(op.in), s, sb) == 0, JN_ESTATE,
                   "launch_spp_bwd: %s was refused (channel block, alignment or LDS)", op.name.c_str());
          break;
        }
        case BR_UPSAMPLE:
          JN_CHECK(launch_upsample_bwd(gptr(op.out), ld(op.out), gptr(op.in), ld(op.in), op.in.C, op.in.H, op.in.W, N, op.acc_in ? 1 : 0, s, sb) == 0,
                   JN_ESTATE, "launch_upsample_bwd: %s was refused", op.name.c_str());
          break;
        default: break;
      }
      prof.mark(obi);
      continue;
    }
    const ConvW& cw = net.convs[op.wslot];
    const ConvB c{op, st, cw, gptr(st.g), ld(st.g), M, net.bconsts + 3 * cw.stat_off, grad_of(ctx, cw.w_dev)};
    hipStream_t ws = s;
    if ((rc = bn_sums_consts(c))) return rc;
    switch (st.route) {
      case BR_PW_FUSED: case BR_PW_FUSED_HALVES: {
        const int parts = st.route == BR_PW_FUSED ? 1 : 2, pc = cw.cout / parts;
        for (int part = 0; part < parts; ++part) {
          const int c0 = part * pc;
          PwBwdFusedArgs fa{};
          fa.g = c.g + c0; fa.g_ld = c.g_ld; fa.z = ptr(op.out) + c0; fa.z_ld = ld(op.out); fa.ot = tab_at(tab(op.out), c0);
          fa.save = save + 2 * (cw.stat_off + c0); fa.consts = c.consts + 3 * c0;
          fa.x = ptr(op.in); fa.x_ld = ld(op.in); fa.it = tab(op.in); fa.w = cw.w_dev + (size_t)c0 * cw.cin;
          fa.gx = gptr(op.in); fa.gx_ld = ld(op.in); fa.accumulate = (op.acc_in || part > 0) ? 1 : 0;
          fa.gw = c.gw + (size_t)c0 * cw.cin; fa.wpart = ctx->wpart; fa.M = M; fa.cout = pc; fa.cin = cw.cin; fa.sb = sb;
          if (st.fold >= 0) {
            const View& sum = net.ops[st.fold].out;
            fa.gadd = gptr(sum); fa.gadd_ld = ld(sum); fa.accumulate = 0;
          }
          if (st.red_in >= 0 || st.red_in2 >= 0) fa.red_rep_stride = rep_stride;
          if (st.red_in >= 0) fa.red_in = sums(st.red_in, st.red_half);
          if (st.red_in2 >= 0) fa.red_in2 = sums(st.red_in2, st.red_half2);
          fa.red_split = st.red_split;
          if (st.red2) {
            const Op& co = net.ops[st.red_in];
            const ChanTab zt = tab(co.out);
            fa.red2_z = ptr(co.out); fa.red2_ld = ld(co.out); fa.red2_sc = zt.sc; fa.red2_sh = zt.sh;
          }
          if (ctx->params_x3t && cw.cin == 128 && (pc == 128 || pc == 64) && (fa.w - ctx->params) % 8 == 0)
            fa.w_frag = reinterpret_cast<float*>(ctx->params_x3t + 3 * (fa.w - ctx->params));
          JN_CHECK(launch_pw_bwd_fused(fa, s) == 0, JN_ESTATE, "launch_pw_bwd_fused: %s has no kernel, or its LDS was refused", op.name.c_str());
        }
        break;
      }
      case BR_DW_FUSED: {
        DwBwdFusedArgs fa{};
        fa.g = c.g; fa.g_ld = c.g_ld; fa.z = ptr(op.out); fa.z_ld = ld(op.out); fa.ot = tab(op.out);
        fa.save = save + 2 * cw.stat_off; fa.consts = c.consts;
        fa.x = ptr(op.in); fa.x_ld = ld(op.in); fa.it = tab(op.in); fa.w = cw.w_dev;
        fa.gin = gptr(op.in); fa.gin_ld = ld(op.in); fa.accumulate = op.acc_in ? 1 : 0; fa.gw = c.gw; fa.wpart = ctx->wpart;
        fa.C = cw.cout; fa.H = op.in.H; fa.W = op.in.W; fa.OH = op.out.H; fa.OW = op.out.W; fa.N = N; fa.stride = op.stride;
        fa.sb = sb;
        if (st.red_in >= 0) {
          fa.red_in = sums(st.red_in, st.red_half); fa.red_rep_stride = rep_stride;
          fa.accumulate = 0;
        }
        JN_CHECK(launch_dw_bwd_fused(fa, s) == 0, JN_ESTATE, "launch_dw_bwd_fused: %s has no kernel", op.name.c_str());
        break;
      }
      case BR_STEM_FUSED:
        JN_CHECK(launch_stem_bwd_weight(stem_args(ss, net, N, cw), c.g, c.g_ld, c.gw, ctx->wpart, s, sb, ptr(op.out), ld(op.out), tab(op.out),
                                        save + 2 * cw.stat_off, c.consts) == 0,
                 JN_ESTATE, "launch_stem_bwd_weight: %s was refused (patch size %d, %d output channels)", op.name.c_str(), net.P, cw.cout);
        break;
      case BR_PW: {
        bn_gz(c);
        const ConvArgs a = gz_conv_args(c);
        if (cw.cout >= 128 && cw.cin >= 128 && (rc = fork_aux(ws))) return rc;
        const bool x3 = !std::getenv("JN_NO_PW_X3_BWD") && !op.acc_in && ctx->params_x3t &&
                        pw_x3_bwd_data_supported(cw.cout, cw.cin) && (cw.w_dev - ctx->params) % 8 == 0;
        if (!x3 || launch_pw_x3_bwd_data(a, cw.w_dev, ctx->params_x3t + 3 * (cw.w_dev - ctx->params), s) != 0)
          JN_CHECK(launch_pw(a, s) == 0, JN_ESTATE, "data gradient of %s: no kernel for this shape, or its LDS was refused", op.name.c_str());
        JN_CHECK(launch_pw_bwd_weight(c.g, c.g_ld, ptr(op.in), ld(op.in), tab(op.in), c.gw, ctx->wpart, M, cw.cout, cw.cin, ws, sb) == 0,
                 JN_ESTATE, "launch_pw_bwd_weight: %s has no kernel, or its LDS was refused", op.name.c_str());
        break;
      }
      case BR_DW:
        bn_gz(c);
        launch_dw_bwd_data(c.g, c.g_ld, cw.w_dev, gptr(op.in), ld(op.in), cw.cout, op.in.H, op.in.W, op.out.H, op.out.W, N, op.stride,
                           op.acc_in ? 1 : 0, s, sb);
        launch_dw_bwd_weight(c.g, c.g_ld, ptr(op.in), ld(op.in), tab(op.in), c.gw, ctx->wpart, cw.cout, op.in.H, op.in.W, op.out.H,
                             op.out.W, N, op.stride, s, sb);
        break;
      case BR_CONV3_S1: case BR_CONV3_S2: {
        bn_gz(c);
        if ((rc = fork_aux(ws))) return rc;
        const int rc3 = st.route == BR_CONV3_S1
                            ? launch_conv3(gz_conv_args(c), s, 0)
                            : launch_conv3_bwd_data_s2(c.g, c.g_ld, cw.w_dev, gptr(op.in), ld(op.in), op.in.H, op.in.W, op.out.H,
                                                       op.out.W, cw.cout, cw.cin, N, op.acc_in ? 1 : 0, s, sb, 0);
        JN_CHECK(rc3 == 0, JN_ESTATE, "backward of dense 3x3 conv %s: unsupported shape", op.name.c_str());
        JN_CHECK(launch_conv3_bwd_weight(c.g, c.g_ld, ptr(op.in), ld(op.in), tab(op.in), c.gw, op.in.H, op.in.W, op.out.H, op.out.W,
                                         cw.cout, cw.cin, N, op.stride, ws, sb, 0, 0) == 0,
                 JN_ESTATE, "launch_conv3_bwd_weight: the LDS of %s was refused", op.name.c_str());
        break;
      }
      default: JN_CHECK(false, JN_ESTATE, "backward plan: conv %s has route %d", op.name.c_str(), (int)st.route);
    }
    prof.mark(obi);
  }
  if (aux_used) {
    JN_HIP(hipEventRecord(ctx->aux_join, ctx->aux_stream));
    JN_HIP(hipStreamWaitEvent(s, ctx->aux_join, 0));
  }
  if (prof) {
    (void)hipStreamSynchronize(s);
    fprintf(stderr, "# backward profile: net %d, N=%d patches x %d steps; bytes = g_out + z_out + x read, g_in written (+ read when accumulated)\n", ni, N, nsl);
    for (int obi = n_ops_b - 1; obi >= 0; --obi) {
      const Op& op = net.ops[obi];
      const double in_e = op.kind == OP_STEM ? 0.0 : (double)op.in.H * op.in.W * op.in.C, out_e = (double)op.out.H * op.out.W * op.out.C;
      double elems;
      if (op.wslot >= 0) elems = 2.0 * out_e + (op.kind == OP_STEM ? 3.0 * net.P * net.P : 2.0 * in_e + (op.acc_in ? in_e : 0.0));
      else if (op.kind == OP_ADDACT) elems = 3.0 * out_e;
      else if (op.kind == OP_SPP) elems = 8.0 * in_e;
      else elems = in_e + out_e;
      prof.row(op, obi + 1, obi, elems * 4.0 * N * nsl, true);
    }
    prof.total();
  }
  JN_HIP(hipGetLastError());
  return JN_OK;
}

int run_embed_fpn(jn_ctx* ctx, int N, int slot, float* e_buf, const int* skip_flag, int skip_when, hipStream_t s, int tab_slot) {
  if (!e_buf) e_buf = ctx->efpn_act;
  const Net& net = ctx->nets[ctx->enc_net];
  jn_ctx& x = *ctx;
  const int C = ctx->cfg.n_embd, MB = ctx->cfg.max_batch;
  const View& f = net.fpn[2];
  ConvArgs a{};
  a.in = view_ptr(net, slot, MB, f); a.in_ld = net.bufs[f.buf].C; a.in_dtype = net.act_dtype; a.itab = view_tab(net, tab_slot < 0 ? slot : tab_slot, f);
  a.out_dtype = JN_F32; a.bf16_mfma = net.act_dtype == JN_BF16;
  a.w = ctx->gpt.efpn_w; a.bias = nullptr; a.out = e_buf; a.out_ld = C;
  a.N = N; a.H = f.H; a.W = f.W; a.OH = f.H; a.OW = f.W; a.cin = f.C; a.cout = C; a.stride = 1; a.act = ACT_RELU;
  a.skip_flag = skip_flag; a.skip_when = skip_when;
  JN_CHECK(launch_pw(a, s) == 0, JN_ESTATE, "embed_fpn.0: no kernel for this shape, or its LDS was refused");
  JN_CHECK(launch_efpn_linear(e_buf, ctx->gpt.efpn_lin_wt, x.emb_part, N, f.H * f.W * C, C, x.KS, skip_flag, skip_when, s) == 0, JN_ESTATE,
           "embed_fpn.3: no kernel for %d outputs", C);
  JN_HIP(hipGetLastError());
  return JN_OK;
}

int replay_slot_diff(jn_ctx* ctx, Net& net, int slot_a, int slot_b, int N, long long* n_diff, hipStream_t s) {
  const int MB = ctx->cfg.max_batch;
  JN_CHECK(slot_a >= 0 && slot_b >= 0 && slot_a < net.a_slots && slot_b < net.a_slots && N >= 1 && N <= MB, JN_ESTATE,
           "compare of activation slots %d and %d over %d patches: not allocated", slot_a, slot_b, N);
  JN_CHECK(net.act_dtype == JN_F32, JN_ESTATE, "the slot compare reads fp32 activations");
  unsigned long long* total = nullptr;
  JN_HIP(hipMalloc((void**)&total, sizeof(unsigned long long)));
  hipError_t e = hipMemsetAsync(total, 0, sizeof(unsigned long long), s);
  for (size_t b = 0; b < net.bufs.size() && e == hipSuccess; ++b) {
    View v; v.buf = (int)b; v.coff = 0;
    const long long n = (long long)N * (long long)net.bufs[b].per_image();
    if (n == 0) continue;
    const unsigned grid = (unsigned)std::min<long long>((n + 255) / 256, 2048);
    hipLaunchKernelGGL(word_diff_kernel, dim3(grid), dim3(256), 0, s, (const uint32_t*)view_ptr(net, slot_a, MB, v),
                       (const uint32_t*)view_ptr(net, slot_b, MB, v), n, total);
  }
  unsigned long long host = 0;
  if (e == hipSuccess) e = hipGetLastError();
  if (e == hipSuccess) e = hipMemcpyAsync(&host, total, sizeof(host), hipMemcpyDeviceToHost, s);
  if (e == hipSuccess) e = hipStreamSynchronize(s);
  (void)hipFree(total);
  JN_HIP(e);
  *n_diff = (long long)host;
  return JN_OK;
}

int embed_tokens(jn_ctx* ctx, const StemSrc& ss, int N, int train, float* e_buf, float* out, long long out_stride,
                 hipStream_t s) {
  int rc;
  if ((rc = run_net(ctx, ctx->enc_net, N, ss, 0, train, nullptr, 0, s))) return rc;
  if ((rc = run_embed_fpn(ctx, N, 0, e_buf, nullptr, 0, s))) return rc;
  const int C = ctx->cfg.n_embd;
  hipLaunchKernelGGL(emb_finish_kernel, dim3((N * C + 255) / 256), dim3(256), 0, s, ctx->emb_part, ctx->gpt.efpn_lin_b, out,
                     out_stride, N, ctx->KS, C);
  return JN_OK;
}

static int check_net_batch(const jn_ctx* ctx, int net, int N) {
  JN_CHECK(net >= 0 && net < 2 && ctx->has_net[net], JN_EINVAL, "network %d is not part of this context", net);
  JN_CHECK(ctx->weights_loaded, JN_ESTATE, "jn_load_weights has not been called");
  JN_CHECK(N >= 1 && N <= ctx->cfg.max_batch, JN_EINVAL, "N=%d exceeds max_batch=%d", N, ctx->cfg.max_batch);
  return JN_OK;
}

}

extern "C" {

int jn_debug_forward_plan(const jn_ctx* ctx, int net, int N, int train, int with_head, int first_op, int32_t* out, int cap) {
  JN_CHECK(ctx && net >= 0 && net < 2 && ctx->has_net[net] && (out || cap <= 0), JN_EINVAL, "jn_debug_forward_plan: bad argument");
  const Net& n = ctx->nets[net];
  std::vector<FwdStep> plan;
  const int rc = plan_forward(n, N, train != 0, with_head != 0, first_op, train && !with_head && defer_eligible(n), plan);
  if (rc) return rc;
  for (int i = 0; i < (int)plan.size() && i < cap; ++i) {
    out[3 * i] = plan[i].route; out[3 * i + 1] = plan[i].link; out[3 * i + 2] = plan[i].deferred;
  }
  return (int)plan.size();
}

int jn_backbone_forward(jn_ctx* ctx, int net, const float* patches_dev, int N, int train, float* fpn0_dev,
                        float* fpn1_dev, float* fpn2_dev, void* stream) {
  JN_CHECK(ctx && patches_dev, JN_EINVAL, "jn_backbone_forward: null argument");
  int rc = check_net_batch(ctx, net, N);
  if (rc) return rc;
  JN_HIP(hipSetDevice(ctx->cfg.device));
  hipStream_t s = (hipStream_t)stream;
  if ((rc = run_net(ctx, net, N, patch_src(patches_dev, ctx->cfg.patch_size), 0, train ? 1 : 0, nullptr, 0, s))) return rc;
  float* outs[3] = {fpn0_dev, fpn1_dev, fpn2_dev};
  const Net& n = ctx->nets[net];
  for (int i = 0; i < 3; ++i) {
    if (!outs[i]) continue;
    const View& f = n.fpn[i];
    launch_nhwc_to_nchw(view_ptr(n, 0, ctx->cfg.max_batch, f), n.act_dtype, n.bufs[f.buf].C, view_tab(n, 0, f), outs[i], f.C,
                        f.H * f.W, N, s);
  }
  JN_HIP(hipGetLastError());
  return JN_OK;
}

int jn_backbone_backward(jn_ctx* ctx, int net, const float* patches_dev, int N, const float* g0_dev,
                         const float* g1_dev, const float* g2_dev, void* stream) {
  JN_CHECK(ctx && patches_dev, JN_EINVAL, "jn_backbone_backward: null argument");
  int rc = check_net_batch(ctx, net, N);
  if (rc) return rc;
  Net& n = ctx->nets[net];
  JN_CHECK(n.act_dtype == JN_F32, JN_ESTATE, "training needs act_dtype = fp32 (bf16 is the inference mode)");
  JN_HIP(hipSetDevice(ctx->cfg.device));
  if ((rc = ensure_train_state(ctx))) return rc;
  hipStream_t s = (hipStream_t)stream;
  const int MB = ctx->cfg.max_batch;
  const float* gs[3] = {g0_dev, g1_dev, g2_dev};
  int fpn_zero = 0;
  for (int i = 0; i < 3; ++i) {
    const View& f = n.fpn[i];
    float* gp = n.gact + n.buf_off[f.buf] * (size_t)MB + f.coff;
    if (gs[i]) {
      launch_nchw_to_nhwc_grad(gs[i], gp, n.bufs[f.buf].C, f.C, f.H * f.W, N, 0, s);
    } else {
      JN_CHECK(n.bufs[f.buf].C == f.C, JN_ESTATE, "fpn output is a slice");
      JN_HIP(hipMemsetAsync(gp, 0, (size_t)N * f.H * f.W * f.C * sizeof(float), s));
      fpn_zero |= 1 << i;
    }
  }
  return run_net_backward(ctx, net, N, patch_src(patches_dev, ctx->cfg.patch_size), 0, s, 1, 0, false, fpn_zero);
}

int jn_embed_patches(jn_ctx* ctx, const float* patches_dev, int N, float* out_dev, void* stream) {
  JN_CHECK(ctx && patches_dev && out_dev, JN_EINVAL, "jn_embed_patches: null argument");
  JN_CHECK(!ctx->cfg.no_patch_emb, JN_ESTATE, "context was created with no_patch_emb");
  int rc = check_net_batch(ctx, ctx->enc_net, N);
  if (rc) return rc;
  JN_HIP(hipSetDevice(ctx->cfg.device));
  if ((rc = embed_tokens(ctx, patch_src(patches_dev, ctx->cfg.patch_size), N, 0, nullptr, out_dev, ctx->cfg.n_embd, (hipStream_t)stream)))
    return rc;
  JN_HIP(hipGetLastError());
  return JN_OK;
}

}
```

jolineedle_amd/csrc/kernels_bwd_pw.hip:

```cpp
#include <hip/hip_runtime.h>

#include <algorithm>
#include <cstdlib>

#include "jn_kernels.h"
#include "jn_reduce.h"
#include "jn_split.h"
#include "jn_tab.h"
#include "jn_types.h"

namespace jnr {

constexpr int WG_RB = 64;

template <int CTN, int CTK>
__global__ __launch_bounds__(256) void pw_bwd_weight_kernel(const float* __restrict__ gz, int g_ld,
                                                            const float* __restrict__ x, int x_ld, ChanTab it,
                                                            float* __restrict__ gw, int rep, long long M, int N,
                                                            int K, int rows_per_block, int chunks_per_slot,
                                                            long long gz_slot, long long x_slot, long long tab_slot) {
  constexpr int LDN = 16 * CTN + 4, LDK = 16 * CTK + 4;
  const int slot = blockIdx.x / chunks_per_slot, chunk = blockIdx.x - slot * chunks_per_slot;
  gz += slot * gz_slot; x += slot * x_slot;
  it.sc += slot * tab_slot; it.sh += slot * tab_slot; it.fl += slot * tab_slot;
// ... 234 lines not shown
template <int CTN, int CTK, bool RED, bool RED2 = false>
__global__ __launch_bounds__(256) void pw_bwd_fused_kernel(
    const float* __restrict__ g, int g_ld, const float* __restrict__ z, int z_ld, ChanTab ot,
    const float* __restrict__ save, const float* __restrict__ consts, const float* __restrict__ x, int x_ld,
    ChanTab it, const float* __restrict__ w, float* __restrict__ gx, int gx_ld, int accumulate,
    float* __restrict__ gw, int rep, long long M, SlotBatch sb, double* __restrict__ red_in, long long red_rep_stride,
    const float* __restrict__ gadd, int gadd_ld, double* __restrict__ red_in2, int red_split,
    const float* __restrict__ red2_z, int red2_ld, const float* __restrict__ red2_sc, const float* __restrict__ red2_sh) {
  constexpr int N = 16 * CTN, K = 16 * CTK;
  constexpr int LDG = N + 4, LDA = K + 4, LDW = N + 4;
  constexpr int NG = 64 * (N / 4) / 256, NA = 64 * (K / 4) / 256;
  constexpr int NGq = NG > 0 ? NG : 1, NAq = NA > 0 ? NA : 1;
  extern __shared__ __attribute__((aligned(16))) float sm[];
  float* Gs = sm;
  float* As = Gs + 64 * LDG;
  float* Wt = As + 64 * LDA;
  float* Cs = Wt + K * LDW;
  float* Ts = sm;
  {
    const long long sl = blockIdx.y;
    g += sl * sb.grad; z += sl * sb.act; x += sl * sb.act; gx += sl * sb.grad;
    save += sl * sb.save; consts += sl * sb.consts;
    if (RED) { if (red_in) red_in += sl * sb.red; if (red_in2) red_in2 += sl * sb.red; }
    if (gadd) gadd += sl * sb.grad;
    if constexpr (RED2) { red2_z += sl * sb.act; red2_sc += sl * sb.tab; red2_sh += sl * sb.tab; }
    ot.sc += sl * sb.tab; ot.sh += sl * sb.tab;
    it.sc += sl * sb.tab; it.sh += sl * sb.tab; it.fl += sl * sb.tab;
  }
  const int tid = threadIdx.x, lane = tid & 63, wave = tid >> 6;
  const int lm = lane & 15, gq = lane >> 4;
  for (int i = tid; i < N * K; i += 256) {
    const int n = i / K, k = i - n * K;
    Wt[k * LDW + n] = w[i];
  }
  const int nq = tid % (N / 4), kq = tid % (K / 4);
  for (int c = tid; c < N; c += 256) {
    Cs[c] = ot.sc[c]; Cs[N + c] = ot.sh[c]; Cs[2 * N + c] = save[2 * c]; Cs[3 * N + c] = save[2 * c + 1];
    Cs[4 * N + c] = consts[3 * c]; Cs[5 * N + c] = consts[3 * c + 1]; Cs[6 * N + c] = consts[3 * c + 2];
  }
  for (int c = tid; c < K; c += 256) { Cs[7 * N + c] = it.sc[c]; Cs[7 * N + K + c] = it.sh[c]; Cs[7 * N + 2 * K + c] = it.fl[c]; }
  if (RED) {
    for (int c = tid; c < 8 * K; c += 256) Cs[7 * N + 3 * K + c] = 0.0f;
    if constexpr (RED2)
      for (int c = tid; c < K; c += 256) {
        const bool in = c < red_split;
        Cs[7 * N + 11 * K + c] = in ? red2_sc[c] : 1.0f; Cs[7 * N + 12 * K + c] = in ? red2_sh[c] : 0.0f;
      }
  }
  constexpr bool DW_SPLIT = (CTK % 2 == 0) || (CTN % 2 == 0);
  constexpr bool DW_HALF_K = DW_SPLIT && CTK % 2 == 0;
  constexpr int DW_AN = !DW_SPLIT ? CTN : (DW_HALF_K ? CTN : CTN / 2), DW_BN = !DW_SPLIT ? CTK : (DW_HALF_K ? CTK / 2 : CTK);
  const int dw_a0 = (DW_SPLIT && !DW_HALF_K) ? (wave & 1) * DW_AN : 0, dw_b0 = DW_HALF_K ? (wave & 1) * DW_BN : 0;
  f32x4 dw[DW_AN][DW_BN];
#pragma unroll
  for (int a = 0; a < DW_AN; ++a)
#pragma unroll
    for (int b = 0; b < DW_BN; ++b) dw[a][b] = f32x4{0.f, 0.f, 0.f, 0.f};

  const long long n_tiles = (M + 63) / 64;
  f32x4 rg[NGq], rz[NGq], rx[NAq];
  auto fetch = [&](long long m0) {
#pragma unroll
    for (int j = 0; j < NGq; ++j) {
      const int i = tid + 256 * j, r = i / (N / 4);
      rg[j] = f32x4{0.f, 0.f, 0.f, 0.f}; rz[j] = rg[j];
      if (i < 64 * (N / 4) && m0 + r < M) {
        rg[j] = *reinterpret_cast<const f32x4*>(g + (m0 + r) * g_ld + 4 * nq);
        rz[j] = *reinterpret_cast<const f32x4*>(z + (m0 + r) * z_ld + 4 * nq);
      }
    }
#pragma unroll
    for (int j = 0; j < NAq; ++j) {
      const int i = tid + 256 * j, r = i / (K / 4);
      rx[j] = f32x4{0.f, 0.f, 0.f, 0.f};
      if (i < 64 * (K / 4) && m0 + r < M) rx[j] = *reinterpret_cast<const f32x4*>(x + (m0 + r) * x_ld + 4 * kq);
    }
  };
  auto stage = [&](long long m0) {
#pragma unroll
    for (int j = 0; j < NGq; ++j) {
      const int i = tid + 256 * j, r = i / (N / 4);
      if (i < 64 * (N / 4)) {
        f32x4 v = {0.f, 0.f, 0.f, 0.f};
        if (m0 + r < M) {
          const f32x4 o_sc = *reinterpret_cast<const f32x4*>(Cs + 4 * nq), o_sh = *reinterpret_cast<const f32x4*>(Cs + N + 4 * nq),
                      o_mean = *reinterpret_cast<const f32x4*>(Cs + 2 * N + 4 * nq), o_istd = *reinterpret_cast<const f32x4*>(Cs + 3 * N + 4 * nq),
                      o_c1 = *reinterpret_cast<const f32x4*>(Cs + 4 * N + 4 * nq), o_c2 = *reinterpret_cast<const f32x4*>(Cs + 5 * N + 4 * nq),
                      o_k = *reinterpret_cast<const f32x4*>(Cs + 6 * N + 4 * nq);
#pragma unroll
          for (int q = 0; q < 4; ++q) {
            const float zh = (rz[j][q] - o_mean[q]) * o_istd[q];
            const float gy = rg[j][q] * dsilu_(fmaf(rz[j][q], o_sc[q], o_sh[q]));
            v[q] = o_k[q] * (gy - o_c1[q] - zh * o_c2[q]);
          }
        }
        *reinterpret_cast<f32x4*>(Gs + r * LDG + 4 * nq) = v;
      }
    }
#pragma unroll
    for (int j = 0; j < NAq; ++j) {
      const int i = tid + 256 * j, r = i / (K / 4);
      if (i < 64 * (K / 4)) {
        f32x4 v = {0.f, 0.f, 0.f, 0.f};
        if (m0 + r < M) {
          if constexpr (RED) v = rx[j];
          else v = tf4(rx[j], *reinterpret_cast<const f32x4*>(Cs + 7 * N + 4 * kq), *reinterpret_cast<const f32x4*>(Cs + 7 * N + K + 4 * kq),
                       *reinterpret_cast<const f32x4*>(Cs + 7 * N + 2 * K + 4 * kq));
        }
        *reinterpret_cast<f32x4*>(As + r * LDA + 4 * kq) = v;
      }
    }
  };

  float p_sc[RED ? CTK : 1], p_sh[RED ? CTK : 1], p_fl[RED ? CTK : 1];
  if constexpr (RED) {
#pragma unroll
    for (int b = 0; b < CTK; ++b) { p_sc[b] = it.sc[16 * b + lm]; p_sh[b] = it.sh[16 * b + lm]; p_fl[b] = it.fl[16 * b + lm]; }
  }
  long long tile = blockIdx.x;
  if (tile < n_tiles) fetch(tile * 64);
  for (; tile < n_tiles; tile += gridDim.x) {
    const long long m0 = tile * 64;
    __syncthreads();
    stage(m0);
    __syncthreads();
    if (tile + gridDim.x < n_tiles) fetch((tile + gridDim.x) * 64);
    {
      f32x4 acc[CTK];
#pragma unroll
      for (int b = 0; b < CTK; ++b) acc[b] = f32x4{0.f, 0.f, 0.f, 0.f};
      f32x4 z2v[RED2 ? CTK : 1];
      if constexpr (RED2) {
        const long long mz = m0 + wave * 16 + lm;
#pragma unroll
        for (int b = 0; b < CTK; ++b) {
          z2v[b] = f32x4{0.f, 0.f, 0.f, 0.f};
          if (16 * b < red_split && mz < M) z2v[b] = *reinterpret_cast<const f32x4*>(red2_z + mz * red2_ld + 16 * b + 4 * gq);
        }
      }
      const float* grow = Gs + (wave * 16 + lm) * LDG + 4 * gq;
      const float* wrow = Wt + lm * LDW + 4 * gq;
#pragma unroll
      for (int kk = 0; kk < N; kk += 16) {
        const f32x4 gb = *reinterpret_cast<const f32x4*>(grow + kk);
#pragma unroll
        for (int b = 0; b < CTK; ++b) {
          const f32x4 wa = *reinterpret_cast<const f32x4*>(wrow + b * 16 * LDW + kk);
#pragma unroll
          for (int j = 0; j < 4; ++j) acc[b] = __builtin_amdgcn_mfma_f32_16x16x4f32(wa[j], gb[j], acc[b], 0, 0, 0);
        }
      }
      const long long m = m0 + wave * 16 + lm;
      if (m < M) {
#pragma unroll
        for (int b = 0; b < CTK; ++b) {
          float* op = gx + m * gx_ld + 16 * b + 4 * gq;
          f32x4 v = acc[b];
          if (gadd) v += *reinterpret_cast<const f32x4*>(gadd + m * gadd_ld + 16 * b + 4 * gq);
          if (accumulate) v += *reinterpret_cast<const f32x4*>(op);
          *reinterpret_cast<f32x4*>(op) = v;
          acc[b] = v;
        }
      }
      if constexpr (RED) {
        float* rslot = Cs + 7 * N + 3 * K + wave * 2 * K;
#pragma unroll
        for (int b = 0; b < CTK; ++b) {
          const int ch = 16 * b + 4 * gq;
          f32x4 zv = *reinterpret_cast<const f32x4*>(As + (wave * 16 + lm) * LDA + ch);
          f32x4 i_sc = *reinterpret_cast<const f32x4*>(Cs + 7 * N + ch), i_sh = *reinterpret_cast<const f32x4*>(Cs + 7 * N + K + ch);
          if constexpr (RED2) if (16 * b < red_split) {
            zv = z2v[b];
            i_sc = *reinterpret_cast<const f32x4*>(Cs + 7 * N + 11 * K + ch); i_sh = *reinterpret_cast<const f32x4*>(Cs + 7 * N + 12 * K + ch);
          }
#pragma unroll
          for (int q = 0; q < 4; ++q) {
            const float yv = fmaf(zv[q], i_sc[q], i_sh[q]);
            const float gy = m < M ? acc[b][q] * dsilu_(yv) : 0.0f;
            const float a1 = row16_sum(gy);
            const float a2 = row16_sum(gy * yv);
            if (lm == 0) { rslot[2 * (ch + q)] += a1; rslot[2 * (ch + q) + 1] += a2; }
          }
        }
      }
    }
    if constexpr (DW_SPLIT) {
      const int prow = 32 * (wave >> 1) + 4 * gq;
      bf16x8 bh[DW_BN], bl[DW_BN];
#pragma unroll
      for (int b = 0; b < DW_BN; ++b)
#pragma unroll
        for (int e = 0; e < 8; ++e) {
          float v = As[(prow + (e & 3) + 16 * (e >> 2)) * LDA + 16 * (dw_b0 + b) + lm];
          if constexpr (RED) v = p_fl[dw_b0 + b] != 0.0f ? silu(fmaf(v, p_sc[dw_b0 + b], p_sh[dw_b0 + b])) : v;
          split2(v, bh[b], bl[b], e);
        }
#pragma unroll
      for (int a = 0; a < DW_AN; ++a) {
        bf16x8 ah, al;
#pragma unroll
        for (int e = 0; e < 8; ++e) {
          const float v = Gs[(prow + (e & 3) + 16 * (e >> 2)) * LDG + 16 * (dw_a0 + a) + lm];
          split2(v, ah, al, e);
        }
#pragma unroll
        for (int b = 0; b < DW_BN; ++b) {
          f32x4 d = dw[a][b];
          d = __builtin_amdgcn_mfma_f32_16x16x32_bf16(ah, bh[b], d, 0, 0, 0);
          d = __builtin_amdgcn_mfma_f32_16x16x32_bf16(ah, bl[b], d, 0, 0, 0);
          d = __builtin_amdgcn_mfma_f32_16x16x32_bf16(al, bh[b], d, 0, 0, 0);
          dw[a][b] = d;
        }
      }
    } else {
#pragma unroll
      for (int st = 0; st < 4; ++st) {
        const int row = wave * 16 + 4 * st + gq;
        float av[CTN], bv[CTK];
#pragma unroll
        for (int a = 0; a < CTN; ++a) av[a] = Gs[row * LDG + 16 * a + lm];
#pragma unroll
        for (int b = 0; b < CTK; ++b) {
          bv[b] = As[row * LDA + 16 * b + lm];
          if constexpr (RED) bv[b] = p_fl[b] != 0.0f ? silu(fmaf(bv[b], p_sc[b], p_sh[b])) : bv[b];
        }
#pragma unroll
        for (int a = 0; a < CTN; ++a)
#pragma unroll
          for (int b = 0; b < CTK; ++b) dw[a][b] = __builtin_amdgcn_mfma_f32_16x16x4f32(av[a], bv[b], dw[a][b], 0, 0, 0);
      }
    }
  }
  if constexpr (RED) {
    __syncthreads();
    const float* rs = Cs + 7 * N + 3 * K;
    if (tid < 2 * K) {
      const bool first = tid < 2 * red_split;
      double* base = first ? red_in : red_in2;
      if (base)
        atomicAdd(&base[(blockIdx.x % JN_NREP) * red_rep_stride + (first ? tid : tid - 2 * red_split)],
                  (double)(rs[tid] + rs[2 * K + tid] + rs[4 * K + tid] + rs[6 * K + tid]));
    }
  }
  if constexpr (DW_SPLIT) {
    for (int ph = 0; ph < 2; ++ph) {
      __syncthreads();
      if ((wave >> 1) == ph) {
#pragma unroll
        for (int a = 0; a < DW_AN; ++a)
#pragma unroll
          for (int b = 0; b < DW_BN; ++b)
#pragma unroll
            for (int r = 0; r < 4; ++r) {
              float* tp = &Ts[(16 * (dw_a0 + a) + 4 * gq + r) * K + 16 * (dw_b0 + b) + lm];
              *tp = (ph == 0 ? 0.0f : *tp) + dw[a][b][r];
            }
      }
    }
  } else {
    for (int wv = 0; wv < 4; ++wv) {
      __syncthreads();
      if (wave == wv) {
#pragma unroll
        for (int a = 0; a < DW_AN; ++a)
#pragma unroll
          for (int b = 0; b < DW_BN; ++b)
#pragma unroll
            for (int r = 0; r < 4; ++r) {
              float* tp = &Ts[(16 * a + 4 * gq + r) * K + 16 * b + lm];
              *tp = (wv == 0 ? 0.0f : *tp) + dw[a][b][r];
            }
      }
    }
  }
  __syncthreads();
  float* dst = rep ? gw + ((blockIdx.x + 5 * blockIdx.y) % JN_NREP) * JN_WPART_MAX : gw;
  for (int i = tid; i < N * K; i += 256) atomicAdd(&dst[i], Ts[i]);
}

template <int CTN, int CTK, bool RED, bool RED2 = false>
static int launch_pw_bwd_fused_r(const PwBwdFusedArgs& a, hipStream_t s) {
  constexpr int N = 16 * CTN, K = 16 * CTK;
  constexpr size_t tiles = ((size_t)64 * (N + 4) + 64 * (K + 4) + (size_t)K * (N + 4) + 7 * N + 3 * K + (RED ? (RED2 ? 10 : 8) * K : 0)) * sizeof(float);
  constexpr size_t smem = std::max(tiles, (size_t)N * K * sizeof(float));
  if (!allow_lds<&pw_bwd_fused_kernel<CTN, CTK, RED, RED2>>(smem)) return -1;
  const long long n_tiles = (a.M + 63) / 64;
  const int places = resident_per_cu<&pw_bwd_fused_kernel<CTN, CTK, RED, RED2>>(smem, 2) * JN_NUM_CU;
  const int rounds = std::max(1, (1024 + places / 2) / places);
  long long bx = (long long)rounds * places / a.sb.n;
  if (a.max_wg > 0 && bx > a.max_wg / a.sb.n) bx = a.max_wg / a.sb.n;
  if (bx < 1) bx = 1;
  if (bx > n_tiles) bx = n_tiles;
  const int rep = (a.wpart && N * K <= JN_WPART_MAX) ? 1 : 0;
  hipLaunchKernelGGL((pw_bwd_fused_kernel<CTN, CTK, RED, RED2>), dim3((unsigned)bx, a.sb.n), dim3(256), smem, s, a.g, a.g_ld, a.z,
                     a.z_ld, a.ot, a.save, a.consts, a.x, a.x_ld, a.it, a.w, a.gx, a.gx_ld, a.accumulate,
                     rep ? a.wpart : a.gw, rep, a.M, a.sb, a.red_in, a.red_rep_stride, a.gadd, a.gadd_ld, a.red_in2,
                     a.red_split > 0 ? a.red_split : K, a.red2_z, a.red2_ld, a.red2_sc, a.red2_sh);
  if (rep) launch_wpart_reduce(a.gw, a.wpart, N * K, s);
  return 0;
}

template <int CTN, int CTK>
static int launch_pw_bwd_fused_t(const PwBwdFusedArgs& a, hipStream_t s) {
  if constexpr (CTK <= 4) {
    if (a.red2_z) return launch_pw_bwd_fused_r<CTN, CTK, true, true>(a, s);
    if (a.red_in || a.red_in2) return launch_pw_bwd_fused_r<CTN, CTK, true>(a, s);
  }
  return launch_pw_bwd_fused_r<CTN, CTK, false>(a, s);
}


using gfloat_p = const __attribute__((address_space(1))) float*;
__device__ __forceinline__ gfloat_p pin_uniform(const float* p) {
  asm volatile("" : "+s"(p));
  return (gfloat_p)p;
}
__device__ __forceinline__ f32x4 ldg4(gfloat_p base, unsigned off) {
  return *(const __attribute__((address_space(1))) f32x4*)(base + off);
}

__global__ __launch_bounds__(256) void w_frag_t_kernel(const float* __restrict__ w, float* __restrict__ wf, int N, int K) {
  const int i = blockIdx.x * 256 + threadIdx.x;
  if (i >= N * K / 4) return;
  const int lane = i & 63, lm = lane & 15, gq = lane >> 4, NS = N / 16, s = (i >> 6) % NS, b = (i >> 6) / NS;
  f32x4 v;
#pragma unroll
  for (int j = 0; j < 4; ++j) v[j] = w[(long long)(16 * s + 4 * gq + j) * K + 16 * b + lm];
  *reinterpret_cast<f32x4*>(wf + 4LL * i) = v;
}

template <int CTN, int D, bool X3>
__global__ __launch_bounds__(256, 2) void pw_bwd_fused128_kernel(
    const float* __restrict__ g, int g_ld, const float* __restrict__ z, int z_ld, ChanTab ot,
    const float* __restrict__ save, const float* __restrict__ consts, const float* __restrict__ x, int x_ld,
    ChanTab it, const float* __restrict__ wf, float* __restrict__ gx, int gx_ld, int accumulate,
    float* __restrict__ gw, int rep, long long M, SlotBatch sb, const float* __restrict__ gadd, int gadd_ld) {
  constexpr int N = 16 * CTN, K = 128, NS = N / 16;
  constexpr int LDG = N + 4, LDA = K + 4;
  constexpr int NG = 32 * (N / 4) / 256, NA = 32 * (K / 4) / 256;
  constexpr int NJ = N / 32, LDK = N + 16;
  static_assert(NG >= 1 && D >= 1 && D < (X3 ? 2 * NJ : NS), "pw_bwd_fused128 tile mapping");
  constexpr int TILE = 32 * LDG + 32 * LDA, NBUF = X3 ? 1 : 2;
  __shared__ __attribute__((aligned(16))) float sm[NBUF * TILE + 7 * N + 3 * K + (X3 ? 3 * 32 * LDK / 2 : 0)];
  float* Gs = sm;
  float* As = Gs + 32 * LDG;
  float* const Cs = sm + NBUF * TILE;
  bf16_t* const Gp = reinterpret_cast<bf16_t*>(Cs + 7 * N + 3 * K);
  const int tid = threadIdx.x, lane = tid & 63, wave = tid >> 6;
  const int lm = lane & 15, gq = lane >> 4;
  const int nq = tid % (N / 4), kq = tid % (K / 4);
  const long long tiles_per_slot = (M + 31) / 32, n_tiles = tiles_per_slot * sb.n;
  const long long t_begin = n_tiles * blockIdx.x / gridDim.x, t_end = n_tiles * (blockIdx.x + 1) / gridDim.x;
  if (t_begin >= t_end) return;

  constexpr int DW_AN = CTN / 2, DW_BN = 4;
  const int dw_a0 = (wave & 1) * DW_AN, dw_b0 = (wave >> 1) * DW_BN;
  f32x4 dw[DW_AN][DW_BN];
#pragma unroll
  for (int a = 0; a < DW_AN; ++a)
#pragma unroll
    for (int b = 0; b < DW_BN; ++b) dw[a][b] = f32x4{0.f, 0.f, 0.f, 0.f};

  f32x4 rg[NG], rz[NG], rx[NA];
  long long f_slot = 0, f_m0 = 0;
  auto fetch = [&](bool next) {
    if (next) {
      f_m0 += 32;
      if (f_m0 >= M) { f_m0 = 0; ++f_slot; }
    }
    const gfloat_p gs = pin_uniform(g + f_slot * sb.grad + f_m0 * g_ld), zs = pin_uniform(z + f_slot * sb.act + f_m0 * z_ld),
                   xs = pin_uniform(x + f_slot * sb.act + f_m0 * x_ld);
    const int last = (int)(M - f_m0 < 32 ? M - f_m0 : 32) - 1;
#pragma unroll
    for (int j = 0; j < NG; ++j) {
      const int r = std::min((tid + 256 * j) / (N / 4), last);
      rg[j] = ldg4(gs, r * g_ld + 4 * nq);
      rz[j] = ldg4(zs, r * z_ld + 4 * nq);
    }
#pragma unroll
    for (int j = 0; j < NA; ++j) {
      const int r = std::min((tid + 256 * j) / (K / 4), last);
      rx[j] = ldg4(xs, r * x_ld + 4 * kq);
    }
  };
  f32x4 eo[2][2];
  auto fetch_store_operand = [&](long long slot, long long m0) {
    const gfloat_p src = pin_uniform(gadd ? gadd + slot * sb.grad + m0 * gadd_ld : gx + slot * sb.grad + m0 * gx_ld);
    const int src_ld = gadd ? gadd_ld : gx_ld;
    const int last = (int)(M - m0 < 32 ? M - m0 : 32) - 1;
#pragma unroll
    for (int c = 0; c < 2; ++c)
#pragma unroll
      for (int p = 0; p < 2; ++p)
        eo[c][p] = ldg4(src, std::min(16 * p + lm, last) * src_ld + 16 * (2 * wave + c) + 4 * gq);
  };
  auto load_consts = [&](long long sl) {
    const gfloat_p o_sc = pin_uniform(ot.sc + sl * sb.tab), o_sh = pin_uniform(ot.sh + sl * sb.tab), sv = pin_uniform(save + sl * sb.save),
                   cn = pin_uniform(consts + sl * sb.consts);
    for (int c = tid; c < N; c += 256) {
      Cs[c] = o_sc[c]; Cs[N + c] = o_sh[c]; Cs[2 * N + c] = sv[2 * c]; Cs[3 * N + c] = sv[2 * c + 1];
      Cs[4 * N + c] = cn[3 * c]; Cs[5 * N + c] = cn[3 * c + 1]; Cs[6 * N + c] = cn[3 * c + 2];
    }
    const gfloat_p i_sc = pin_uniform(it.sc + sl * sb.tab), i_sh = pin_uniform(it.sh + sl * sb.tab), i_fl = pin_uniform(it.fl + sl * sb.tab);
    for (int c = tid; c < K; c += 256) { Cs[7 * N + c] = i_sc[c]; Cs[7 * N + K + c] = i_sh[c]; Cs[7 * N + 2 * K + c] = i_fl[c]; }
  };
  auto stage = [&](long long m0) {
#pragma unroll
    for (int j = 0; j < NG; ++j) {
      const int r = (tid + 256 * j) / (N / 4);
      f32x4 v = {0.f, 0.f, 0.f, 0.f};
      if (m0 + r < M) {
        const f32x4 o_sc = *reinterpret_cast<const f32x4*>(Cs + 4 * nq), o_sh = *reinterpret_cast<const f32x4*>(Cs + N + 4 * nq),
                    o_mean = *reinterpret_cast<const f32x4*>(Cs + 2 * N + 4 * nq), o_istd = *reinterpret_cast<const f32x4*>(Cs + 3 * N + 4 * nq),
                    o_c1 = *reinterpret_cast<const f32x4*>(Cs + 4 * N + 4 * nq), o_c2 = *reinterpret_cast<const f32x4*>(Cs + 5 * N + 4 * nq),
                    o_k = *reinterpret_cast<const f32x4*>(Cs + 6 * N + 4 * nq);
#pragma unroll
        for (int q = 0; q < 4; ++q) {
          const float zh = (rz[j][q] - o_mean[q]) * o_istd[q];
          const float gy = rg[j][q] * dsilu_(fmaf(rz[j][q], o_sc[q], o_sh[q]));
          v[q] = o_k[q] * (gy - o_c1[q] - zh * o_c2[q]);
        }
      }
      *reinterpret_cast<f32x4*>(Gs + r * LDG + 4 * nq) = v;
      if constexpr (X3) {
        const bf16x4 vh = __builtin_convertvector(v, bf16x4);
        const f32x4 r1 = v - __builtin_convertvector(vh, f32x4);
        const bf16x4 vm = __builtin_convertvector(r1, bf16x4);
        const f32x4 r2 = r1 - __builtin_convertvector(vm, f32x4);
        bf16_t* dst = Gp + r * LDK + 4 * nq;
        *reinterpret_cast<bf16x4*>(dst) = vh;
        *reinterpret_cast<bf16x4*>(dst + 32 * LDK) = vm;
        *reinterpret_cast<bf16x4*>(dst + 2 * 32 * LDK) = __builtin_convertvector(r2, bf16x4);
      }
    }
#pragma unroll
    for (int j = 0; j < NA; ++j) {
      const int r = (tid + 256 * j) / (K / 4);
      f32x4 v = {0.f, 0.f, 0.f, 0.f};
      if (m0 + r < M)
        v = tf4(rx[j], *reinterpret_cast<const f32x4*>(Cs + 7 * N + 4 * kq), *reinterpret_cast<const f32x4*>(Cs + 7 * N + K + 4 * kq),
                *reinterpret_cast<const f32x4*>(Cs + 7 * N + 2 * K + 4 * kq));
      *reinterpret_cast<f32x4*>(As + r * LDA + 4 * kq) = v;
    }
  };

  gfloat_p wbase = pin_uniform(wf);
  const unsigned woff = (2 * wave * NS * 64 + lane) * 4;
  auto wfrag = [&](int c, int s) -> f32x4 { return ldg4(wbase, woff + (c * NS + s) * 256); };
  auto wfrag3 = [&](int c, int j, int t) -> bf16x8 {
    return __builtin_bit_cast(bf16x8, ldg4(wbase, (((2 * wave + c) * NJ + j) * 3 + t) * 256 + lane * 4));
  };

  long long cur_slot = -1;
  f_slot = t_begin / tiles_per_slot;
  f_m0 = (t_begin - f_slot * tiles_per_slot) * 32;
  fetch(false);
#pragma unroll 1
  for (long long tile = t_begin; tile < t_end; ++tile) {
    const long long slot = f_slot, m0 = f_m0;
    f32x4 wa[X3 ? 1 : NS][2];
    bf16x8 wx[X3 ? 2 * NJ : 1][3];
    wbase = pin_uniform(wf);
#pragma unroll
    for (int s = 0; s < D; ++s) {
      if constexpr (X3) {
#pragma unroll
        for (int t = 0; t < 3; ++t) wx[s][t] = wfrag3(s & 1, s >> 1, t);
      } else {
#pragma unroll
        for (int c = 0; c < 2; ++c) wa[s][c] = wfrag(c, s);
      }
    }
    if constexpr (NBUF == 1) __syncthreads();
    if (slot != cur_slot) {
      load_consts(slot);
      cur_slot = slot;
      __syncthreads();
    }
    if constexpr (NBUF == 2) {
      Gs = sm + ((tile - t_begin) & 1) * TILE;
      As = Gs + 32 * LDG;
    }
    stage(m0);
    __syncthreads();
    f32x4 acc[2][2];
#pragma unroll
    for (int c = 0; c < 2; ++c)
#pragma unroll
      for (int p = 0; p < 2; ++p) acc[c][p] = f32x4{0.f, 0.f, 0.f, 0.f};
    auto late_loads = [&]() {
      if (gadd || accumulate) fetch_store_operand(slot, m0);
      fetch(tile + 1 < t_end);
    };
    if constexpr (X3) {
      const bf16_t* xrow = Gp + lm * LDK + 8 * gq;
#pragma unroll
      for (int u = 0; u < 2 * NJ; ++u) {
        const int j = u >> 1, c = u & 1;
        if (u + D < 2 * NJ) {
#pragma unroll
          for (int t = 0; t < 3; ++t) wx[u + D][t] = wfrag3((u + D) & 1, (u + D) >> 1, t);
        }
        if (u + D == 2 * NJ - 1) late_loads();
        __builtin_amdgcn_sched_barrier(0);
#pragma unroll
        for (int p = 0; p < 2; ++p) {
          bf16x8 xa[3];
#pragma unroll
          for (int t = 0; t < 3; ++t) xa[t] = *reinterpret_cast<const bf16x8*>(xrow + t * 32 * LDK + p * 16 * LDK + 32 * j);
#pragma unroll
          for (int e = 0; e < X3_PRODUCTS; ++e) acc[c][p] = __builtin_amdgcn_mfma_f32_16x16x32_bf16(wx[u][X3_W[e]], xa[X3_X[e]], acc[c][p], 0, 0, 0);
        }
      }
    } else {
      const float* grow = Gs + lm * LDG + 4 * gq;
#pragma unroll
      for (int s = 0; s < NS; ++s) {
        if (s + D < NS) {
#pragma unroll
          for (int c = 0; c < 2; ++c) wa[s + D][c] = wfrag(c, s + D);
        }
        if (s + D == NS - 1) late_loads();
        __builtin_amdgcn_sched_barrier(0);
        f32x4 gb[2];
#pragma unroll
        for (int p = 0; p < 2; ++p) gb[p] = *reinterpret_cast<const f32x4*>(grow + p * 16 * LDG + 16 * s);
#pragma unroll
        for (int c = 0; c < 2; ++c)
#pragma unroll
          for (int p = 0; p < 2; ++p)
#pragma unroll
            for (int j = 0; j < 4; ++j) acc[c][p] = __builtin_amdgcn_mfma_f32_16x16x4f32(wa[s][c][j], gb[p][j], acc[c][p], 0, 0, 0);
      }
    }
    {
      float* gxs = gx + slot * sb.grad + m0 * gx_ld;
#pragma unroll
      for (int c = 0; c < 2; ++c)
#pragma unroll
        for (int p = 0; p < 2; ++p)
          if (m0 + 16 * p + lm < M) {
            float* op = gxs + (unsigned)((16 * p + lm) * gx_ld + 16 * (2 * wave + c) + 4 * gq);
            f32x4 v = acc[c][p];
            if (gadd || accumulate) v += eo[c][p];
            if (gadd && accumulate) v += *reinterpret_cast<const f32x4*>(op);
            *reinterpret_cast<f32x4*>(op) = v;
          }
    }
    {
      const int prow = 4 * gq;
      bf16x8 bh[DW_BN], bl[DW_BN];
#pragma unroll
      for (int b = 0; b < DW_BN; ++b)
#pragma unroll
        for (int e = 0; e < 8; ++e) {
          const float v = As[(prow + (e & 3) + 16 * (e >> 2)) * LDA + 16 * (dw_b0 + b) + lm];
          split2(v, bh[b], bl[b], e);
        }
#pragma unroll
      for (int a = 0; a < DW_AN; ++a) {
        bf16x8 ah, al;
#pragma unroll
        for (int e = 0; e < 8; ++e) {
          const float v = Gs[(prow + (e & 3) + 16 * (e >> 2)) * LDG + 16 * (dw_a0 + a) + lm];
          split2(v, ah, al, e);
        }
#pragma unroll
        for (int b = 0; b < DW_BN; ++b) {
          f32x4 d = dw[a][b];
          d = __builtin_amdgcn_mfma_f32_16x16x32_bf16(ah, bh[b], d, 0, 0, 0);
          d = __builtin_amdgcn_mfma_f32_16x16x32_bf16(ah, bl[b], d, 0, 0, 0);
          d = __builtin_amdgcn_mfma_f32_16x16x32_bf16(al, bh[b], d, 0, 0, 0);
          dw[a][b] = d;
        }
      }
    }
  }
  float* dst = rep ? gw + (blockIdx.x % JN_NREP) * JN_WPART_MAX : gw;
#pragma unroll
  for (int a = 0; a < DW_AN; ++a)
#pragma unroll
    for (int b = 0; b < DW_BN; ++b)
#pragma unroll
      for (int r = 0; r < 4; ++r) atomicAdd(&dst[(16 * (dw_a0 + a) + 4 * gq + r) * K + 16 * (dw_b0 + b) + lm], dw[a][b][r]);
}

template <int CTN, int D, bool X3>
static void launch_pw_bwd_fused128(const PwBwdFusedArgs& a, hipStream_t s) {
  constexpr int N = 16 * CTN, K = 128;
  if (X3) launch_w_split3_t(a.w, a.w_frag, N, K, s);
  else hipLaunchKernelGGL(w_frag_t_kernel, dim3(N * K / 4 / 256), dim3(256), 0, s, a.w, a.w_frag, N, K);
  const int places = resident_per_cu<&pw_bwd_fused128_kernel<CTN, D, X3>>(0, 2) * JN_NUM_CU;
  const long long n_tiles = (a.M + 31) / 32 * a.sb.n;
  long long bx = std::min<long long>(places, n_tiles);
  if (a.max_wg > 0) bx = std::min<long long>(bx, a.max_wg);
  const int rep = (a.wpart && N * K <= JN_WPART_MAX) ? 1 : 0;
  hipLaunchKernelGGL((pw_bwd_fused128_kernel<CTN, D, X3>), dim3((unsigned)bx), dim3(256), 0, s, a.g, a.g_ld, a.z, a.z_ld, a.ot, a.save,
                     a.consts, a.x, a.x_ld, a.it, a.w_frag, a.gx, a.gx_ld, a.accumulate, rep ? a.wpart : a.gw, rep, a.M, a.sb,
                     a.gadd, a.gadd_ld);
  if (rep) launch_wpart_reduce(a.gw, a.wpart, N * K, s);
}

static bool pw_bwd_fused128_takes(const PwBwdFusedArgs& a) {
  return a.w_frag && a.route != 1 && a.cin == 128 && (a.cout == 128 || a.cout == 64) && !a.red_in && !a.red_in2 && !a.red2_z &&
         a.g_ld % 4 == 0 && a.z_ld % 4 == 0 && a.x_ld % 4 == 0 && a.gx_ld % 4 == 0 && (!a.gadd || a.gadd_ld % 4 == 0) &&
         reinterpret_cast<uintptr_t>(a.w_frag) % 16 == 0;
}

bool pw_bwd_fused_reduces_input(int cout, int cin) { return pw_bwd_fused_supported(cout, cin) && cin <= 64; }

bool pw_bwd_fused_supported(int cout, int cin) {
  if (cout % 16 || cin % 16) return false;
  const int tn = cout / 16, tk = cin / 16;
  auto pow2 = [](int v) { return v == 1 || v == 2 || v == 4 || v == 8; };
  return pow2(tn) && pow2(tk);
}

int launch_pw_bwd_fused(const PwBwdFusedArgs& a, hipStream_t s) {
  const int tn = a.cout / 16, tk = a.cin / 16;
  if (pw_bwd_fused128_takes(a)) {
    if (tn == 8) launch_pw_bwd_fused128<8, 2, true>(a, s); else launch_pw_bwd_fused128<4, 2, false>(a, s);
    return 0;
  }
#define JN_PF(A, B) if (tn == A && tk == B) return launch_pw_bwd_fused_t<A, B>(a, s);
  JN_PF(1, 1) JN_PF(1, 2) JN_PF(1, 4) JN_PF(1, 8) JN_PF(2, 1) JN_PF(2, 2) JN_PF(2, 4) JN_PF(2, 8)
  JN_PF(4, 1) JN_PF(4, 2) JN_PF(4, 4) JN_PF(4, 8) JN_PF(8, 1) JN_PF(8, 2) JN_PF(8, 4) JN_PF(8, 8)
#undef JN_PF
  return -1;
}

}
```

Measured before the change: 14040 glimpse-patches/s.

## Fuse input-side BN reduction into 128-channel pointwise backward kernel

Extends the specialised cin=128 pointwise backward kernel with a RED variant. It computes the per-channel sums (dy and dy*y through the SiLU derivative) for the preceding layer's batch-norm backward while it writes gx, and flushes them with double atomics per slot. The planner's reduces_input predicate now accepts cin=128, so those layers can drop the separate reduction pass over gx. The generic template path also enables reduction for CTK=8. The fused kernel does extra loads, atomics and LDS use, and adds sync at slot boundaries, which may reduce occupancy.

```diff
diff --git a/include/jnroll.h b/include/jnroll.h
--- a/include/jnroll.h
+++ b/include/jnroll.h
@@ -92,6 +92,9 @@
 int jn_param_info_at(const jn_ctx* ctx, int index, jn_param_info* out);
 int jn_debug_forward_plan(const jn_ctx* ctx, int net, int N, int train, int with_head, int first_op, int32_t* out,
                           int cap);
+#define JN_BWD_PLAN_FIELDS 13
+int jn_debug_backward_plan(const jn_ctx* ctx, int net, int with_head, int fpn_zero, int32_t* out, int cap, char* names,
+                           int names_cap);
 int jn_debug_decision_route(const jn_ctx* ctx);
 int jn_load_weights(jn_ctx* ctx, const jn_tensor* tensors, size_t n);
 
@@ -262,6 +265,10 @@
 int jn_pw_bwd_fused(const float* g_dev, const float* z_dev, const float* x_dev, const float* tab_dev, const float* save_dev,
                     const float* consts_dev, const float* w_dev, const float* gadd_dev, int accumulate, float* gx_dev,
                     float* gw_dev, int S, long long M, int cout, int cin, int route, int max_wg, void* stream);
+int jn_pw_bwd_fused_red(const float* g_dev, const float* z_dev, const float* x_dev, const float* tab_dev, const float* save_dev,
+                        const float* consts_dev, const float* w_dev, const float* gadd_dev, int accumulate, float* gx_dev,
+                        float* gw_dev, int S, long long M, int cout, int cin, int route, int max_wg, double* red_out_dev,
+                        int red_split, int run_mask, const float* red2_z_dev, const float* red2_tab_dev, void* stream);
 int jn_conv3(const void* in_dev, int in_ld, const float* tab_dev, const float* w_dev, void* out_dev, int out_ld, int N, int H,
              int W, int cin, int cout, int stride, int transposed, int accumulate, double* stats_dev, const int* skip_flag_dev,
              int skip_when, int n_slots, long long in_slot_stride, long long out_slot_stride, int route, void* stream);
diff --git a/jolineedle_amd/_lib.py b/jolineedle_amd/_lib.py
--- a/jolineedle_amd/_lib.py
+++ b/jolineedle_amd/_lib.py
@@ -76,6 +76,7 @@
     "jn_param_count": (C.c_int, [C.c_void_p]),
     "jn_param_info_at": (C.c_int, [C.c_void_p, C.c_int, C.POINTER(JnParamInfo)]),
     "jn_debug_forward_plan": (C.c_int, [C.c_void_p, C.c_int, C.c_int, C.c_int, C.c_int, C.c_int, C.POINTER(C.c_int32), C.c_int]),
+    "jn_debug_backward_plan": (C.c_int, [C.c_void_p, C.c_int, C.c_int, C.c_int, C.POINTER(C.c_int32), C.c_int, C.c_char_p, C.c_int]),
     "jn_debug_decision_route": (C.c_int, [C.c_void_p]),
     "jn_load_weights": (C.c_int, [C.c_void_p, C.POINTER(JnTensor), C.c_size_t]),
     "jn_env_init": (C.c_int, [C.c_void_p, C.c_void_p, C.c_void_p, C.c_int, C.c_int, C.c_int, C.c_int, C.c_int,
@@ -154,6 +155,8 @@
     "jn_teacher_actions": (C.c_int, [C.c_void_p, C.c_void_p, C.c_void_p, C.c_int, C.c_int, C.c_int, C.c_void_p, C.c_void_p]),
     "jn_teacher_walks": (C.c_int, [C.c_void_p, C.c_void_p] + [C.c_int] * 9 + [C.c_uint64, C.c_int] + [C.c_void_p] * 12),
     "jn_pw_bwd_fused": (C.c_int, [C.c_void_p] * 8 + [C.c_int] + [C.c_void_p] * 2 + [C.c_int, C.c_longlong] + [C.c_int] * 4 + [C.c_void_p]),
+    "jn_pw_bwd_fused_red": (C.c_int, [C.c_void_p] * 8 + [C.c_int] + [C.c_void_p] * 2 + [C.c_int, C.c_longlong] + [C.c_int] * 4 +
+                            [C.c_void_p, C.c_int, C.c_int, C.c_void_p, C.c_void_p, C.c_void_p]),
     "jn_conv3": (C.c_int, [C.c_void_p, C.c_int, C.c_void_p, C.c_void_p, C.c_void_p] + [C.c_int] * 9 + [C.c_void_p, C.c_void_p, C.c_int, C.c_int,
                            C.c_longlong, C.c_longlong, C.c_int, C.c_void_p]),
     "jn_conv3_bwd_data_s2": (C.c_int, [C.c_void_p, C.c_int, C.c_void_p, C.c_void_p] + [C.c_int] * 9 + [C.c_void_p]),
diff --git a/jolineedle_amd/csrc/api_kernels.hip b/jolineedle_amd/csrc/api_kernels.hip
--- a/jolineedle_amd/csrc/api_kernels.hip
+++ b/jolineedle_amd/csrc/api_kernels.hip
@@ -58,27 +58,37 @@
   return JN_OK;
 }
 
-extern "C" {
-
-int jn_pw_bwd_fused(const float* g_dev, const float* z_dev, const float* x_dev, const float* tab_dev, const float* save_dev,
-                    const float* consts_dev, const float* w_dev, const float* gadd_dev, int accumulate, float* gx_dev,
-                    float* gw_dev, int S, long long M, int cout, int cin, int route, int max_wg, void* stream) {
-  JN_CHECK(g_dev && z_dev && x_dev && tab_dev && save_dev && consts_dev && w_dev && gx_dev && gw_dev, JN_EINVAL,
-           "jn_pw_bwd_fused: null argument");
-  JN_CHECK(S >= 1 && M >= 1 && M <= (1LL << 40), JN_EINVAL, "jn_pw_bwd_fused: S=%d M=%lld", S, M);
-  JN_CHECK(cout >= 16 && cin >= 16 && pw_bwd_fused_supported(cout, cin), JN_EINVAL, "jn_pw_bwd_fused: %d -> %d channels: no fused kernel",
-           cin, cout);
-  JN_CHECK((route == 0 || route == 1) && max_wg >= 0, JN_EINVAL, "jn_pw_bwd_fused: route=%d max_wg=%d", route, max_wg);
+static int pw_bwd_fused_entry(const char* who, const float* g_dev, const float* z_dev, const float* x_dev, const float* tab_dev,
+                              const float* save_dev, const float* consts_dev, const float* w_dev, const float* gadd_dev, int accumulate,
+                              float* gx_dev, float* gw_dev, int S, long long M, int cout, int cin, int route, int max_wg,
+                              double* red_out_dev, int red_split, int run_mask, const float* red2_z_dev, const float* red2_tab_dev,
+                              void* stream) {
+  JN_CHECK(g_dev && z_dev && x_dev && tab_dev && save_dev && consts_dev && w_dev && gx_dev && gw_dev, JN_EINVAL, "%s: null argument", who);
+  JN_CHECK(S >= 1 && M >= 1 && M <= (1LL << 40), JN_EINVAL, "%s: S=%d M=%lld", who, S, M);
+  JN_CHECK(cout >= 16 && cin >= 16 && pw_bwd_fused_supported(cout, cin), JN_EINVAL, "%s: %d -> %d channels: no fused kernel", who, cin, cout);
+  JN_CHECK((route == 0 || route == 1) && max_wg >= 0, JN_EINVAL, "%s: route=%d max_wg=%d", who, route, max_wg);
+  if (red_out_dev) {
+    JN_CHECK(pw_bwd_fused_reduces_input(cout, cin), JN_EINVAL, "%s: %d -> %d channels: no kernel that reduces its input", who, cin, cout);
+    JN_CHECK(red_split >= 0 && red_split < cin && red_split % 16 == 0 && run_mask >= 1 && run_mask <= (red_split ? 3 : 1), JN_EINVAL,
+             "%s: red_split=%d run_mask=%d", who, red_split, run_mask);
+    JN_CHECK(!red2_z_dev == !red2_tab_dev && (!red2_z_dev || (run_mask & 1)), JN_EINVAL, "%s: the RED2 operands go with the first run", who);
+  }
   hipStream_t s = (hipStream_t)stream;
   const long long C = cout + cin;
-  const size_t zn = (size_t)M * cout, xn = (size_t)M * cin, act = zn + xn, grad = zn + 2 * xn;
+  const int c2 = red_out_dev && red2_z_dev ? (red_split ? red_split : cin) : 0;
+  const size_t zn = (size_t)M * cout, xn = (size_t)M * cin, z2n = (size_t)M * c2, act = zn + xn + z2n, grad = zn + 2 * xn;
   Scratch scratch(s);
-  JN_HIP(scratch.take(((size_t)S * (act + grad) + (size_t)2 * cout * cin) * sizeof(float)));
+  JN_HIP(scratch.take(((size_t)S * (act + grad) + (size_t)2 * cout * cin + (size_t)S * 3 * C) * sizeof(float)));
   float* ws = scratch.as<float>();
-  float *za = ws, *xa = za + zn, *ga = ws + (size_t)S * act, *gxa = ga + zn, *gadda = gxa + xn, *w_frag = ws + (size_t)S * (act + grad);
+  float *za = ws, *xa = za + zn, *z2a = xa + xn, *ga = ws + (size_t)S * act, *gxa = ga + zn, *gadda = gxa + xn,
+        *w_frag = ws + (size_t)S * (act + grad), *tab2 = w_frag + (size_t)2 * cout * cin;
   const SlotLayout lay{S, s};
   JN_HIP(lay.in(za, act, z_dev, zn));
   JN_HIP(lay.in(xa, act, x_dev, xn));
+  if (c2) {
+    JN_HIP(lay.in(z2a, act, red2_z_dev, z2n));
+    JN_HIP(lay.in(tab2, 3 * C, red2_tab_dev, (size_t)2 * c2));
+  }
   JN_HIP(lay.in(ga, grad, g_dev, zn));
   if (accumulate) JN_HIP(lay.in(gxa, grad, gx_dev, xn));
   if (gadd_dev) JN_HIP(lay.in(gadda, grad, gadd_dev, xn));
@@ -93,8 +103,33 @@
   a.sb.n = S; a.sb.act = (long long)act; a.sb.grad = (long long)grad; a.sb.tab = 3 * C; a.sb.save = 2LL * cout; a.sb.consts = 3LL * cout;
   if (gadd_dev) { a.gadd = gadda; a.gadd_ld = cin; }
   a.w_frag = w_frag; a.route = route; a.max_wg = max_wg;
-  return run_entry("jn_pw_bwd_fused", s, [&] { return launch_pw_bwd_fused(a, s); }, "no fused kernel took the launch",
+  if (red_out_dev) {
+    a.sb.red = (long long)JN_NREP * 2 * cin; a.red_rep_stride = 2LL * cin; a.red_split = red_split;
+    if (run_mask & 1) a.red_in = red_out_dev;
+    if (run_mask & 2) a.red_in2 = red_out_dev + 2 * red_split;
+    if (c2) { a.red2_z = z2a; a.red2_ld = c2; a.red2_sc = tab2; a.red2_sh = tab2 + c2; }
+  }
+  return run_entry(who, s, [&] { return launch_pw_bwd_fused(a, s); }, "no fused kernel took the launch",
                    [&] { return lay.back(gx_dev, xn, gxa, grad); });
+}
+
+extern "C" {
+
+int jn_pw_bwd_fused(const float* g_dev, const float* z_dev, const float* x_dev, const float* tab_dev, const float* save_dev,
+                    const float* consts_dev, const float* w_dev, const float* gadd_dev, int accumulate, float* gx_dev,
+                    float* gw_dev, int S, long long M, int cout, int cin, int route, int max_wg, void* stream) {
+  return pw_bwd_fused_entry("jn_pw_bwd_fused", g_dev, z_dev, x_dev, tab_dev, save_dev, consts_dev, w_dev, gadd_dev, accumulate, gx_dev,
+                            gw_dev, S, M, cout, cin, route, max_wg, nullptr, 0, 0, nullptr, nullptr, stream);
+}
+
+int jn_pw_bwd_fused_red(const float* g_dev, const float* z_dev, const float* x_dev, const float* tab_dev, const float* save_dev,
+                        const float* consts_dev, const float* w_dev, const float* gadd_dev, int accumulate, float* gx_dev,
+                        float* gw_dev, int S, long long M, int cout, int cin, int route, int max_wg, double* red_out_dev,
+                        int red_split, int run_mask, const float* red2_z_dev, const float* red2_tab_dev, void* stream) {
+  JN_CHECK(red_out_dev, JN_EINVAL, "jn_pw_bwd_fused_red: null argument");
+  return pw_bwd_fused_entry("jn_pw_bwd_fused_red", g_dev, z_dev, x_dev, tab_dev, save_dev, consts_dev, w_dev, gadd_dev, accumulate,
+                            gx_dev, gw_dev, S, M, cout, cin, route, max_wg, red_out_dev, red_split, run_mask, red2_z_dev, red2_tab_dev,
+                            stream);
 }
 
 }
diff --git a/jolineedle_amd/csrc/api_net.hip b/jolineedle_amd/csrc/api_net.hip
--- a/jolineedle_amd/csrc/api_net.hip
+++ b/jolineedle_amd/csrc/api_net.hip
@@ -772,6 +772,34 @@
   return (int)plan.size();
 }
 
+int jn_debug_backward_plan(const jn_ctx* ctx, int net, int with_head, int fpn_zero, int32_t* out, int cap, char* names, int names_cap) {
+  JN_CHECK(ctx && net >= 0 && net < 2 && ctx->has_net[net] && (out || cap <= 0) && (names || names_cap <= 0) && fpn_zero >= 0 && fpn_zero < 8,
+           JN_EINVAL, "jn_debug_backward_plan: bad argument");
+  const Net& n = ctx->nets[net];
+  std::vector<BwdStep> plan;
+  const int rc = plan_backward(n, with_head != 0, fpn_zero, plan);
+  if (rc) return rc;
+  size_t used = 0;
+  if (names_cap > 0) names[0] = 0;
+  for (int i = 0; i < (int)plan.size(); ++i) {
+    const BwdStep& st = plan[i];
+    const Op& op = n.ops[i];
+    if (i < cap) {
+      const ConvW* cw = op.wslot >= 0 ? &n.convs[op.wslot] : nullptr;
+      const int32_t rec[JN_BWD_PLAN_FIELDS] = {st.route, st.red_in, st.red_half, st.red_in2, st.red_half2, st.red2 ? 1 : 0, st.red_by, st.fold,
+                                               (int32_t)op.kind, cw ? cw->cout : op.out.C, cw ? cw->cin : op.in.C, op.out.H * op.out.W,
+                                               cw && !cw->prefix2.empty() ? 1 : 0};
+      std::memcpy(out + (size_t)JN_BWD_PLAN_FIELDS * i, rec, sizeof rec);
+    }
+    if (used + op.name.size() + 2 <= (size_t)names_cap) {
+      std::memcpy(names + used, op.name.data(), op.name.size());
+      used += op.name.size();
+      names[used++] = '\n'; names[used] = 0;
+    }
+  }
+  return (int)plan.size();
+}
+
 int jn_backbone_forward(jn_ctx* ctx, int net, const float* patches_dev, int N, int train, float* fpn0_dev,
                         float* fpn1_dev, float* fpn2_dev, void* stream) {
   JN_CHECK(ctx && patches_dev, JN_EINVAL, "jn_backbone_forward: null argument");
diff --git a/jolineedle_amd/csrc/kernels_bwd_pw.hip b/jolineedle_amd/csrc/kernels_bwd_pw.hip
--- a/jolineedle_amd/csrc/kernels_bwd_pw.hip
+++ b/jolineedle_amd/csrc/kernels_bwd_pw.hip
@@ -560,7 +560,7 @@
 
 template <int CTN, int CTK>
 static int launch_pw_bwd_fused_t(const PwBwdFusedArgs& a, hipStream_t s) {
-  if constexpr (CTK <= 4) {
+  if constexpr (CTK <= 4 || (CTK == 8 && CTN >= 4)) {
     if (a.red2_z) return launch_pw_bwd_fused_r<CTN, CTK, true, true>(a, s);
     if (a.red_in || a.red_in2) return launch_pw_bwd_fused_r<CTN, CTK, true>(a, s);
   }
@@ -572,6 +572,16 @@
 __device__ __forceinline__ gfloat_p pin_uniform(const float* p) {
   asm volatile("" : "+s"(p));
   return (gfloat_p)p;
+}
+__device__ __forceinline__ gfloat_p pin_wave_uniform(const float* p) {
+  const unsigned long long v = reinterpret_cast<unsigned long long>(p);
+  const unsigned lo = __builtin_amdgcn_readfirstlane((unsigned)v), hi = __builtin_amdgcn_readfirstlane((unsigned)(v >> 32));
+  return (gfloat_p)(((unsigned long long)hi << 32) | lo);
+}
+template <bool OPAQUE>
+__device__ __forceinline__ int opaque_if(int v) {
+  if constexpr (OPAQUE) asm volatile("" : "+v"(v));
+  return v;
 }
 __device__ __forceinline__ f32x4 ldg4(gfloat_p base, unsigned off) {
   return *(const __attribute__((address_space(1))) f32x4*)(base + off);
@@ -587,23 +597,35 @@
   *reinterpret_cast<f32x4*>(wf + 4LL * i) = v;
 }
 
-template <int CTN, int D, bool X3>
+template <bool RED>
+struct PwRed128 {};
+template <>
+struct PwRed128<true> {
+  double* red_in; long long red_rep_stride; double* red_in2; int red_split;
+  const float* red2_z; int red2_ld; const float* red2_sc; const float* red2_sh;
+};
+
+template <int CTN, int D, bool X3, bool RED = false>
 __global__ __launch_bounds__(256, 2) void pw_bwd_fused128_kernel(
     const float* __restrict__ g, int g_ld, const float* __restrict__ z, int z_ld, ChanTab ot,
     const float* __restrict__ save, const float* __restrict__ consts, const float* __restrict__ x, int x_ld,
     ChanTab it, const float* __restrict__ wf, float* __restrict__ gx, int gx_ld, int accumulate,
-    float* __restrict__ gw, int rep, long long M, SlotBatch sb, const float* __restrict__ gadd, int gadd_ld) {
+    float* __restrict__ gw, int rep, long long M, SlotBatch sb, const float* __restrict__ gadd, int gadd_ld,
+    PwRed128<RED> rd) {
   constexpr int N = 16 * CTN, K = 128, NS = N / 16;
   constexpr int LDG = N + 4, LDA = K + 4;
   constexpr int NG = 32 * (N / 4) / 256, NA = 32 * (K / 4) / 256;
   constexpr int NJ = N / 32, LDK = N + 16;
   static_assert(NG >= 1 && D >= 1 && D < (X3 ? 2 * NJ : NS), "pw_bwd_fused128 tile mapping");
   constexpr int TILE = 32 * LDG + 32 * LDA, NBUF = X3 ? 1 : 2;
-  __shared__ __attribute__((aligned(16))) float sm[NBUF * TILE + 7 * N + 3 * K + (X3 ? 3 * 32 * LDK / 2 : 0)];
+  constexpr int PLANES = X3 ? 3 * 32 * LDK / 2 : 0;
+  __shared__ __attribute__((aligned(16))) float sm[NBUF * TILE + 7 * N + 3 * K + PLANES + (RED ? 4 * K : 0)];
   float* Gs = sm;
   float* As = Gs + 32 * LDG;
   float* const Cs = sm + NBUF * TILE;
   bf16_t* const Gp = reinterpret_cast<bf16_t*>(Cs + 7 * N + 3 * K);
+  float* const Rt = Cs + 7 * N + 3 * K + PLANES;
+  float* const Rs = Rt + 2 * K;
   const int tid = threadIdx.x, lane = tid & 63, wave = tid >> 6;
   const int lm = lane & 15, gq = lane >> 4;
   const int nq = tid % (N / 4), kq = tid % (K / 4);
@@ -619,6 +641,17 @@
 #pragma unroll
     for (int b = 0; b < DW_BN; ++b) dw[a][b] = f32x4{0.f, 0.f, 0.f, 0.f};
 
+  if constexpr (RED) Rs[tid] = 0.0f;
+  auto flush_red = [&](long long sl) {
+    if constexpr (RED) {
+      const int t = opaque_if<true>(tid);
+      const bool first = t < 2 * rd.red_split;
+      double* base = first ? rd.red_in : rd.red_in2;
+      if (base) atomicAdd(&base[sl * sb.red + (blockIdx.x % JN_NREP) * rd.red_rep_stride + (first ? t : t - 2 * rd.red_split)], (double)Rs[t]);
+      Rs[t] = 0.0f;
+    }
+  };
+
   f32x4 rg[NG], rz[NG], rx[NA];
   long long f_slot = 0, f_m0 = 0;
   auto fetch = [&](bool next) {
@@ -643,24 +676,46 @@
   };
   f32x4 eo[2][2];
   auto fetch_store_operand = [&](long long slot, long long m0) {
-    const gfloat_p src = pin_uniform(gadd ? gadd + slot * sb.grad + m0 * gadd_ld : gx + slot * sb.grad + m0 * gx_ld);
-    const int src_ld = gadd ? gadd_ld : gx_ld;
-    const int last = (int)(M - m0 < 32 ? M - m0 : 32) - 1;
-#pragma unroll
-    for (int c = 0; c < 2; ++c)
-#pragma unroll
-      for (int p = 0; p < 2; ++p)
-        eo[c][p] = ldg4(src, std::min(16 * p + lm, last) * src_ld + 16 * (2 * wave + c) + 4 * gq);
+    if constexpr (RED) {
+      const int last = (int)(M - m0 < 32 ? M - m0 : 32) - 1;
+#pragma unroll
+      for (int c = 0; c < 2; ++c) {
+        const bool behind = rd.red2_z && 16 * (2 * wave + c) < rd.red_split;
+        const gfloat_p src = pin_wave_uniform(behind ? rd.red2_z + slot * sb.act + m0 * rd.red2_ld : x + slot * sb.act + m0 * x_ld);
+        const int src_ld = behind ? rd.red2_ld : x_ld;
+#pragma unroll
+        for (int p = 0; p < 2; ++p)
+          eo[c][p] = ldg4(src, std::min(16 * p + lm, last) * src_ld + 16 * (2 * wave + c) + 4 * gq);
+      }
+    } else {
+      const gfloat_p src = pin_uniform(gadd ? gadd + slot * sb.grad + m0 * gadd_ld : gx + slot * sb.grad + m0 * gx_ld);
+      const int src_ld = gadd ? gadd_ld : gx_ld;
+      const int last = (int)(M - m0 < 32 ? M - m0 : 32) - 1;
+#pragma unroll
+      for (int c = 0; c < 2; ++c)
+#pragma unroll
+        for (int p = 0; p < 2; ++p)
+          eo[c][p] = ldg4(src, std::min(16 * p + lm, last) * src_ld + 16 * (2 * wave + c) + 4 * gq);
+    }
   };
   auto load_consts = [&](long long sl) {
+    const int t = RED ? opaque_if<RED>(tid) : tid;
     const gfloat_p o_sc = pin_uniform(ot.sc + sl * sb.tab), o_sh = pin_uniform(ot.sh + sl * sb.tab), sv = pin_uniform(save + sl * sb.save),
                    cn = pin_uniform(consts + sl * sb.consts);
-    for (int c = tid; c < N; c += 256) {
+    for (int c = t; c < N; c += 256) {
       Cs[c] = o_sc[c]; Cs[N + c] = o_sh[c]; Cs[2 * N + c] = sv[2 * c]; Cs[3 * N + c] = sv[2 * c + 1];
       Cs[4 * N + c] = cn[3 * c]; Cs[5 * N + c] = cn[3 * c + 1]; Cs[6 * N + c] = cn[3 * c + 2];
     }
     const gfloat_p i_sc = pin_uniform(it.sc + sl * sb.tab), i_sh = pin_uniform(it.sh + sl * sb.tab), i_fl = pin_uniform(it.fl + sl * sb.tab);
-    for (int c = tid; c < K; c += 256) { Cs[7 * N + c] = i_sc[c]; Cs[7 * N + K + c] = i_sh[c]; Cs[7 * N + 2 * K + c] = i_fl[c]; }
+    for (int c = t; c < K; c += 256) { Cs[7 * N + c] = i_sc[c]; Cs[7 * N + K + c] = i_sh[c]; Cs[7 * N + 2 * K + c] = i_fl[c]; }
+    if constexpr (RED) {
+      const gfloat_p r_sc = pin_uniform(rd.red2_z ? rd.red2_sc + sl * sb.tab : it.sc + sl * sb.tab),
+                     r_sh = pin_uniform(rd.red2_z ? rd.red2_sh + sl * sb.tab : it.sh + sl * sb.tab);
+      for (int c = t; c < K; c += 256) {
+        const bool behind = rd.red2_z && c < rd.red_split;
+        Rt[c] = behind ? r_sc[c] : i_sc[c]; Rt[K + c] = behind ? r_sh[c] : i_sh[c];
+      }
+    }
   };
   auto stage = [&](long long m0) {
 #pragma unroll
@@ -705,7 +760,9 @@
   gfloat_p wbase = pin_uniform(wf);
   const unsigned woff = (2 * wave * NS * 64 + lane) * 4;
   auto wfrag = [&](int c, int s) -> f32x4 { return ldg4(wbase, woff + (c * NS + s) * 256); };
+  [[maybe_unused]] unsigned w3off = 0;
   auto wfrag3 = [&](int c, int j, int t) -> bf16x8 {
+    if constexpr (RED) return __builtin_bit_cast(bf16x8, ldg4(wbase, w3off + ((c * NJ + j) * 3 + t) * 256));
     return __builtin_bit_cast(bf16x8, ldg4(wbase, (((2 * wave + c) * NJ + j) * 3 + t) * 256 + lane * 4));
   };
 
@@ -719,6 +776,7 @@
     f32x4 wa[X3 ? 1 : NS][2];
     bf16x8 wx[X3 ? 2 * NJ : 1][3];
     wbase = pin_uniform(wf);
+    if constexpr (RED && X3) w3off = opaque_if<true>(2 * wave * NJ * 3 * 256 + lane * 4);
 #pragma unroll
     for (int s = 0; s < D; ++s) {
       if constexpr (X3) {
@@ -731,6 +789,10 @@
     }
     if constexpr (NBUF == 1) __syncthreads();
     if (slot != cur_slot) {
+      if constexpr (RED) {
+        __syncthreads();
+        if (cur_slot >= 0) flush_red(cur_slot);
+      }
       load_consts(slot);
       cur_slot = slot;
       __syncthreads();
@@ -747,7 +809,7 @@
 #pragma unroll
       for (int p = 0; p < 2; ++p) acc[c][p] = f32x4{0.f, 0.f, 0.f, 0.f};
     auto late_loads = [&]() {
-      if (gadd || accumulate) fetch_store_operand(slot, m0);
+      if (RED || gadd || accumulate) fetch_store_operand(slot, m0);
       fetch(tile + 1 < t_end);
     };
     if constexpr (X3) {
@@ -792,18 +854,44 @@
       }
     }
     {
+      [[maybe_unused]] const int lm_s = opaque_if<RED>(lm);
       float* gxs = gx + slot * sb.grad + m0 * gx_ld;
 #pragma unroll
       for (int c = 0; c < 2; ++c)
 #pragma unroll
         for (int p = 0; p < 2; ++p)
           if (m0 + 16 * p + lm < M) {
-            float* op = gxs + (unsigned)((16 * p + lm) * gx_ld + 16 * (2 * wave + c) + 4 * gq);
+            float* op = gxs + (unsigned)((16 * p + (RED ? lm_s : lm)) * gx_ld + 16 * (2 * wave + c) + 4 * gq);
             f32x4 v = acc[c][p];
-            if (gadd || accumulate) v += eo[c][p];
-            if (gadd && accumulate) v += *reinterpret_cast<const f32x4*>(op);
+            if constexpr (RED) {
+              if (gadd) v += ldg4(pin_uniform(gadd + slot * sb.grad + m0 * gadd_ld), (16 * p + lm_s) * gadd_ld + 16 * (2 * wave + c) + 4 * gq);
+              acc[c][p] = v;
+            } else {
+              if (gadd || accumulate) v += eo[c][p];
+              if (gadd && accumulate) v += *reinterpret_cast<const f32x4*>(op);
+            }
             *reinterpret_cast<f32x4*>(op) = v;
           }
+    }
+    if constexpr (RED) {
+#pragma unroll
+      for (int c = 0; c < 2; ++c) {
+        const int ch = 16 * (2 * wave + c) + 4 * gq;
+        const f32x4 r_sc = *reinterpret_cast<const f32x4*>(Rt + ch), r_sh = *reinterpret_cast<const f32x4*>(Rt + K + ch);
+#pragma unroll
+        for (int q = 0; q < 4; ++q) {
+          float a1 = 0.0f, a2 = 0.0f;
+#pragma unroll
+          for (int p = 0; p < 2; ++p) {
+            const float yv = fmaf(eo[c][p][q], r_sc[q], r_sh[q]);
+            const float gy = m0 + 16 * p + lm < M ? acc[c][p][q] * dsilu_(yv) : 0.0f;
+            a1 += gy; a2 += gy * yv;
+          }
+          a1 = row16_sum(a1); a2 = row16_sum(a2);
+          if (lm == 0) { Rs[2 * (ch + q)] += a1; Rs[2 * (ch + q) + 1] += a2; }
+        }
+      }
+      __builtin_amdgcn_sched_barrier(0);
     }
     {
       const int prow = 4 * gq;
@@ -834,6 +922,7 @@
       }
     }
   }
+  if constexpr (RED) flush_red(cur_slot);
   float* dst = rep ? gw + (blockIdx.x % JN_NREP) * JN_WPART_MAX : gw;
 #pragma unroll
   for (int a = 0; a < DW_AN; ++a)
@@ -843,29 +932,36 @@
       for (int r = 0; r < 4; ++r) atomicAdd(&dst[(16 * (dw_a0 + a) + 4 * gq + r) * K + 16 * (dw_b0 + b) + lm], dw[a][b][r]);
 }
 
-template <int CTN, int D, bool X3>
+template <int CTN, int D, bool X3, bool RED>
 static void launch_pw_bwd_fused128(const PwBwdFusedArgs& a, hipStream_t s) {
   constexpr int N = 16 * CTN, K = 128;
+  PwRed128<RED> rd;
+  if constexpr (RED) rd = {a.red_in, a.red_rep_stride, a.red_in2, a.red_split > 0 ? a.red_split : K, a.red2_z, a.red2_ld, a.red2_sc, a.red2_sh};
   if (X3) launch_w_split3_t(a.w, a.w_frag, N, K, s);
   else hipLaunchKernelGGL(w_frag_t_kernel, dim3(N * K / 4 / 256), dim3(256), 0, s, a.w, a.w_frag, N, K);
-  const int places = resident_per_cu<&pw_bwd_fused128_kernel<CTN, D, X3>>(0, 2) * JN_NUM_CU;
+  const int places = resident_per_cu<&pw_bwd_fused128_kernel<CTN, D, X3, RED>>(0, 2) * JN_NUM_CU;
   const long long n_tiles = (a.M + 31) / 32 * a.sb.n;
   long long bx = std::min<long long>(places, n_tiles);
   if (a.max_wg > 0) bx = std::min<long long>(bx, a.max_wg);
   const int rep = (a.wpart && N * K <= JN_WPART_MAX) ? 1 : 0;
-  hipLaunchKernelGGL((pw_bwd_fused128_kernel<CTN, D, X3>), dim3((unsigned)bx), dim3(256), 0, s, a.g, a.g_ld, a.z, a.z_ld, a.ot, a.save,
+  hipLaunchKernelGGL((pw_bwd_fused128_kernel<CTN, D, X3, RED>), dim3((unsigned)bx), dim3(256), 0, s, a.g, a.g_ld, a.z, a.z_ld, a.ot, a.save,
                      a.consts, a.x, a.x_ld, a.it, a.w_frag, a.gx, a.gx_ld, a.accumulate, rep ? a.wpart : a.gw, rep, a.M, a.sb,
-                     a.gadd, a.gadd_ld);
+                     a.gadd, a.gadd_ld, rd);
   if (rep) launch_wpart_reduce(a.gw, a.wpart, N * K, s);
 }
 
 static bool pw_bwd_fused128_takes(const PwBwdFusedArgs& a) {
-  return a.w_frag && a.route != 1 && a.cin == 128 && (a.cout == 128 || a.cout == 64) && !a.red_in && !a.red_in2 && !a.red2_z &&
+  const bool red = a.red_in || a.red_in2;
+  if (red ? (a.accumulate || a.red_split < 0 || a.red_split > 128 || a.red_split % 16 || (a.red2_z && a.red2_ld % 4)) : a.red2_z != nullptr)
+    return false;
+  return a.w_frag && a.route != 1 && a.cin == 128 && (a.cout == 128 || a.cout == 64) &&
          a.g_ld % 4 == 0 && a.z_ld % 4 == 0 && a.x_ld % 4 == 0 && a.gx_ld % 4 == 0 && (!a.gadd || a.gadd_ld % 4 == 0) &&
          reinterpret_cast<uintptr_t>(a.w_frag) % 16 == 0;
 }
 
-bool pw_bwd_fused_reduces_input(int cout, int cin) { return pw_bwd_fused_supported(cout, cin) && cin <= 64; }
+bool pw_bwd_fused_reduces_input(int cout, int cin) {
+  return pw_bwd_fused_supported(cout, cin) && (cin <= 64 || (cin == 128 && (cout == 128 || cout == 64)));
+}
 
 bool pw_bwd_fused_supported(int cout, int cin) {
   if (cout % 16 || cin % 16) return false;
@@ -877,7 +973,9 @@
 int launch_pw_bwd_fused(const PwBwdFusedArgs& a, hipStream_t s) {
   const int tn = a.cout / 16, tk = a.cin / 16;
   if (pw_bwd_fused128_takes(a)) {
-    if (tn == 8) launch_pw_bwd_fused128<8, 2, true>(a, s); else launch_pw_bwd_fused128<4, 2, false>(a, s);
+    const bool red = a.red_in || a.red_in2;
+    if (tn == 8) { if (red) launch_pw_bwd_fused128<8, 2, true, true>(a, s); else launch_pw_bwd_fused128<8, 2, true, false>(a, s); }
+    else { if (red) launch_pw_bwd_fused128<4, 2, false, true>(a, s); else launch_pw_bwd_fused128<4, 2, false, false>(a, s); }
     return 0;
   }
 #define JN_PF(A, B) if (tn == A && tk == B) return launch_pw_bwd_fused_t<A, B>(a, s);
```

Result: no change. 14080 glimpse-patches/s, median of 6 (+0.2%).
